# conroi/lcpc

Measured on AMD Instinct MI355X. Metric: field-elements committed/sec (whole node), Ligero 2^26 coeffs, higher is better.
Workload: dtype u32 limbs (255-bit prime field Ft255, Montgomery form)

## Files before the change

### lcpc_amd/csrc/ctx.cpp

```cpp
#include "internal.h"
#include <chrono>

using namespace lcpc;

namespace lcpc {


const uint8_t LBL_DT[7] = "$l//DT", LBL_PR[7] = "$l//PR", LBL_PE[7] = "$l//PE", LBL_CO[7] = "$l//CO";

void ctx_ref(lcpc_ctx* c) { c->refs.fetch_add(1); }

static void ctx_free(lcpc_ctx* c) {
  (void)hipSetDevice(c->prm.device);
  comm_release(c);
  for (const NttStep& s : c->ntt) dev_free(s.pack);
  dev_free(c->d_wq_w); dev_free(c->d_rootsls); dev_free(c->d_rootslcs);
  dev_free(c->d_rootsl); dev_free(c->d_rootslc); dev_free(c->d_qpl); dev_free(c->d_roots); dev_free(c->d_r2);
  dev_free(c->ws.d_tmp); dev_free(c->ws.d_t); dev_free(c->ws.d_mid); dev_free(c->d_scratch);
  c->verify_sets.clear();
  if (c->s_verify) (void)hipStreamDestroy(c->s_verify);
  for (unsigned k = 0; k < lcpc_ctx::N_STAGE; k++) {
    if (c->h_stage[k]) (void)hipHostFree(c->h_stage[k]);
    if (c->ev_stage[k]) (void)hipEventDestroy(c->ev_stage[k]);
  }
  for (auto* v : {&c->d_pre, &c->d_post})
    for (auto& d : *v) { dev_free(d.rowptr); dev_free(d.colidx); dev_free(d.vals); dev_free(d.vals29); }
  delete c;
}
void ctx_unref(lcpc_ctx* c) {
  if (c->refs.fetch_sub(1) == 1) ctx_free(c);
}

uint64_t ntt_mid_rows(const lcpc_ctx* c, uint64_t n_rows) {
  const bool ev = c->sw_ntt_mid_max_mb >= 0;
  if (c->ntt.size() != 2 || c->ntt[0].kernel != NttStep::K1S || n_rows == 0) return 0;
  if (!ev && c->log_n > 15) return 0;
  const uint64_t max_mb = ev ? (uint64_t)c->sw_ntt_mid_max_mb : 6144;
  if (max_mb == 0) return 0;
  const uint64_t per_row = c->n_cols * 36;
  uint64_t fit = (max_mb << 20) / per_row;
  if (fit == 0) return 0;
  if (fit >= n_rows) return n_rows;
  const uint64_t batches = (n_rows + fit - 1) / fit;
  return (n_rows + batches - 1) / batches;
}

static void wmul_table(const FieldDesc& f, const uint64_t* w_mont, int N, int W, uint32_t out[96]) {
  uint64_t v[MAXL];
  h_canon(f, v, w_mont);
  memset(out, 0, 96 * 4);
  for (int j = 0; j < N; j++) {
    uint64_t m[5] = {0, 0, 0, 0, 0};
    for (int i = 0; i < f.L; i++) m[i] = v[i];
    bool big = false;
    for (int i = f.L - 1; i >= 0; i--) {
      const uint64_t h = (f.p[i] >> 1) | (i + 1 < f.L ? f.p[i + 1] << 63 : 0);
      if (v[i] != h) { big = v[i] > h; break; }
    }
    if (big) {
      unsigned __int128 br = 0;
      for (int i = 0; i < 5; i++) { const unsigned __int128 d = (unsigned __int128)m[i] - (i < f.L ? f.p[i] : 0) - (uint64_t)br; m[i] = (uint64_t)d; br = (d >> 64) & 1; }
    }
    for (int k = 0; k < N; k++) {
      const int b = W * k, wd = b / 64, sh = b % 64;
      uint64_t x = m[wd] >> sh;
      if (sh && wd + 1 < 5) x |= m[wd + 1] << (64 - sh);
      out[N * k + j] = k < N - 1 ? (uint32_t)(x & (((uint64_t)1 << W) - 1)) : (uint32_t)x;
    }
    for (int s = 0; s < W; s++) h_add(f, v, v, v);
  }
}
static int build_wq_w(lcpc_ctx* c, int N, int W) {
  const FieldDesc* f = c->f;
  uint64_t i4[MAXL];
  memcpy(i4, f->rou, 8 * f->L);
  for (unsigned i = 0; i + 2 < f->S; i++) h_mul(*f, i4, i4, i4);
  uint32_t wt[96];
  wmul_table(*f, i4, N, W, wt);
  int rc = dev_alloc(&c->err, &c->d_wq_w, sizeof wt);
  if (rc) return rc;
  HIPCHK(c, hipMemcpy(c->d_wq_w, wt, sizeof wt, hipMemcpyHostToDevice));
  return 0;
}

static std::vector<uint32_t> clamp_table(const FieldDesc& f, int N, int W, int stride) {
  std::vector<uint32_t> tab((size_t)64 * stride, 0);
  for (int i = 0; i < 64; i++) {
    const int q = i - 24;
    uint64_t mag[5] = {0, 0, 0, 0, 0};
    unsigned __int128 cy = 0;
    for (int w = 0; w < 5; w++) { cy += (unsigned __int128)(w < f.L ? f.p[w] : 0) * (uint64_t)(q < 0 ? -q : q); mag[w] = (uint64_t)cy; cy >>= 64; }
    if (q < 0) {
      unsigned __int128 c2 = 1;
      for (int w = 0; w < 5; w++) { c2 += (unsigned __int128)(~mag[w]); mag[w] = (uint64_t)c2; c2 >>= 64; }
    }
    for (int l = 0; l < N; l++) {
      const int b = W * l, w = b / 64, sh = b % 64;
      uint64_t x = mag[w] >> sh;
      if (sh && w + 1 < 5) x |= mag[w + 1] << (64 - sh);
      tab[(size_t)i * stride + l] = l + 1 < N ? (uint32_t)(x & (((uint64_t)1 << W) - 1)) : (uint32_t)x;
    }
  }
  return tab;
}
static int limb_consts(lcpc_ctx* c, std::vector<uint32_t**>* made) {
  const int N = ntt_lns_limbs(c->NL), W = ntt_lns_limb_bits(c->NL);
  const std::vector<uint32_t> tab = clamp_table(*c->f, N, W, ntt_lns_stride(c->NL));
  if (made) { made->push_back(&c->d_qpl); made->push_back(&c->d_wq_w); }
  if (int rc = dev_alloc(&c->err, &c->d_qpl, tab.size() * 4)) return rc;
  HIPCHK(c, hipMemcpy(c->d_qpl, tab.data(), tab.size() * 4, hipMemcpyHostToDevice));
  return build_wq_w(c, N, W);
}

static void plan_passes(lcpc_ctx* c) {
  const unsigned k = c->log_n;
  const int NL = c->NL;
  const int lt_small = NL >= 6 ? 10 : (NL == 4 ? 11 : 12);
  const int lt_big = NL >= 6 ? 11 : 12;
  unsigned ltj_min = 0;
  while (((size_t)NL * 4 << ltj_min) < 128) ltj_min++;
  c->ntt.clear();
  auto add = [&](unsigned t0, unsigned s, unsigned log_tj, int lt) {
    NttStep p;
    p.log_tile = lt;
    p.a.roots = c->d_roots; p.a.roots29 = c->d_rootsl; p.a.qp29 = c->d_qpl; p.a.wq_w = c->d_wq_w;
    p.a.log_n = k; p.a.t0 = t0; p.a.s = s; p.a.log_tj = log_tj;
    p.roots29c = c->d_rootslc;
    p.mont_prefix = t0 + s == k ? (k == 0 ? 1u : (s % 2 == 0 ? 4u : 2u)) : 0u;
    c->ntt.push_back(p);
  };
  if ((int)k <= lt_small) {
    add(0, k, 0, lt_small);
    return;
  }
  int LT = lt_small;
  auto n_pass = [&](int lt) { unsigned per = lt - ltj_min, rest = k - lt; return 1 + (rest + per - 1) / per; };
  if (c->L == 4 && (k == 19 || k == 20) && !c->sw_ntt_general) {
    add(0, k - 10, 20 - k, 10);
    add(k - 10, 10, 0u, 10);
    return;
  }
  if (n_pass(lt_small) > 2 && n_pass(lt_big) < n_pass(lt_small)) LT = lt_big;
  const unsigned P = n_pass(LT);
  const unsigned s_final = LT;
  unsigned rem = k - s_final, t0 = 0;
  for (unsigned i = 0; i + 1 < P; i++) {
    const unsigned left = P - 1 - i;
    const unsigned s = (rem + left - 1) / left;
    add(t0, s, (uint32_t)LT - s, LT);
    t0 += s;
    rem -= s;
  }
  add(t0, s_final, 0u, LT);
}

static uint32_t ntt_tile_group_of(uint32_t log_n, int L, uint32_t log_tj) {
  const uint32_t tiles_log = log_n - 10;
  if (tiles_log < 3) return 0;
  uint32_t run_log = log_tj;
  for (uint32_t b = 8u * (uint32_t)L; b > 1; b >>= 1) run_log++;
  uint32_t lg = run_log <= 5 ? 11 - run_log : (run_log < 10 ? 10 - run_log : 0);
  return std::min(std::min(lg, 6u), tiles_log - 3);
}

static int build_limb_plan(lcpc_ctx* c, unsigned n_pass) {
  std::vector<uint32_t**> made;
  std::vector<NttStep> plan(n_pass);
  const int rc = [&]() -> int {
    const FieldDesc* f = c->f;
    ErrText* err = &c->err;
    const unsigned k = c->log_n, s0 = k - 10 * (n_pass - 1);
    const size_t stride = (size_t)ntt_lns_stride(c->NL);
    auto alloc = [&](uint32_t** p, size_t bytes) { made.push_back(p); return dev_alloc(err, p, bytes); };
    int r;
    if (c->L != 4) {
      uint64_t rp[2 * MAXL] = {1, 0, 0, 0};
      for (int i = 0; i < ntt_lns_limbs(c->NL) * ntt_lns_limb_bits(c->NL); i++) h_add(*f, rp, rp, rp);
      h_canon(*f, rp + f->L, rp);
      const size_t n_roots = (size_t)1 << (k - 1);
      uint32_t* d_rp = nullptr;
      if ((r = dev_alloc(err, &d_rp, 16 * f->L))) return r;
      if ((r = alloc(&c->d_rootsl, n_roots * stride * 4)) || (r = alloc(&c->d_rootslc, n_roots * stride * 4))) { dev_free(d_rp); return r; }
      hipError_t he = hipMemcpy(d_rp, rp, 16 * f->L, hipMemcpyHostToDevice);
      if (he == hipSuccess) he = launch_ntt_lns_roots(c->NL, c->d_roots, n_roots, d_rp, c->d_rootsl, nullptr);
      if (he == hipSuccess) he = launch_ntt_lns_roots(c->NL, c->d_roots, n_roots, d_rp + 2 * f->L, c->d_rootslc, nullptr);
      if (he == hipSuccess) he = hipDeviceSynchronize();
      dev_free(d_rp);
      if (he != hipSuccess) return fail_hip(err, he, "ntt_lns tables");
      if ((r = limb_consts(c, &made))) return r;
    }
    if (n_pass == 3) {
      const size_t n_sub = (size_t)1 << 19;
      if ((r = alloc(&c->d_rootsls, n_sub * stride * 4)) || (r = alloc(&c->d_rootslcs, n_sub * stride * 4))) return r;
      for (int i = 0; i < 2; i++) {
        const uint32_t* tab = i ? c->d_rootslc : c->d_rootsl;
        uint32_t* sub = i ? c->d_rootslcs : c->d_rootsls;
        HIPCHK(c, launch_ntt_lns_subtable(c->NL, tab, s0, n_sub, sub, nullptr));
      }
    }
    for (unsigned i = 0; i < n_pass; i++) {
      NttStep& p = plan[i];
      const bool sub = n_pass == 3 && i > 0, last = i + 1 == n_pass;
      p.kernel = c->L == 4 ? NttStep::K1S : NttStep::K1N;
      p.first = !last;
      p.a.roots = c->d_roots; p.a.roots29 = sub ? c->d_rootsls : c->d_rootsl; p.a.qp29 = c->d_qpl; p.a.wq_w = c->d_wq_w;
      p.a.log_n = sub ? 20u : k;
      p.a.t0 = last ? p.a.log_n - 10 : 0u;
      p.a.s = i == 0 ? s0 : 10u;
      p.a.log_tj = 10 - p.a.s;
      p.a.tile_group = p.first ? ntt_tile_group_of(p.a.log_n, c->L, p.a.log_tj) : 0u;
      p.a.canon_row_mask = sub ? (1u << (k - 20)) - 1 : 0u;
      p.roots29c = sub ? c->d_rootslcs : c->d_rootslc;
      p.mont_prefix = last && c->NL == 2 ? 4u : 0u;
      p.blk0_gone = last && c->NL != 2 && plan[i - 1].a.s >= 8 ? 1u : 0u;
      p.pack_info = ntt_lns_pack_info(c->NL, p.a.s, p.first);
      const uint32_t n_classes = p.first ? 1u << (p.a.log_n - 10) : 1u;
#ifdef LCPC_TEST_HOOKS
      if (n_pass == 3 && i == 0 && c->sw_test_fail_3pass) return LCPC_ERR_NOMEM;
#endif
      if ((r = alloc(&p.pack, (size_t)n_classes * p.pack_info.class_words * 4))) return r;
      NttPassArgs pa{};
      pa.roots29 = p.a.roots29; pa.roots29c = p.roots29c; pa.log_n = p.a.log_n; pa.t0 = p.a.t0; pa.s = p.a.s; pa.log_tj = p.a.log_tj;
      HIPCHK(c, launch_ntt_lns_pack(c->NL, pa, p.first, p.pack_info, n_classes, p.pack, nullptr));
    }
    HIPCHK(c, hipDeviceSynchronize());
    return 0;
  }();
  if (rc == 0) {
    c->ntt = std::move(plan);
    c->comm_canon = true;
    return 0;
  }
  for (uint32_t** p : made) { dev_free(*p); *p = nullptr; }
  if (rc != LCPC_ERR_NOMEM) return rc;
  (void)hipGetLastError();
  c->err.clear();
  return 0;
}

#define ECHK(call)                                                        \
  do {                                                                    \
    hipError_t e__ = (call);                                              \
    if (e__ != hipSuccess) return fail_hip(err, e__, #call);              \
  } while (0)

template <class Mat, class Rs> static int sdig_walk(const lcpc_ctx* c, Mat&& mat, Rs&& rs) {
  const size_t t = c->d_pre.size();
  const DevCsr& pl = c->d_pre[t - 1];
  uint64_t in_start = 0;
  for (size_t i = 0; i + 1 < t; i++) {
    if (int rc = mat(c->d_pre[i], in_start, in_start + c->d_pre[i].n_in, false)) return rc;
    in_start += c->d_pre[i].n_in;
  }
  if (int rc = mat(pl, in_start, 0, true)) return rc;
  const uint64_t in_end = in_start + pl.n_in;
  if (int rc = rs(in_end, c->d_post[t - 1].n_in)) return rc;
  in_start = in_end + pl.n_out;
  uint64_t out_start = in_end + c->d_post[t - 1].n_in;
  for (size_t ii = t; ii-- > 0;) {
    in_start -= c->d_pre[ii].n_out;
    if (int rc = mat(c->d_post[ii], in_start, out_start, false)) return rc;
    out_start += c->d_post[ii].n_out;
  }
  return 0;
}

int encode_rows_device(const lcpc_ctx* c, EncodeWs* ws, const EncodeJob& j, hipStream_t st, ErrText* err, uint32_t* launches) {
  uint32_t dummy = 0;
  uint32_t& nl = launches ? *launches : dummy;
  if (j.kept_t) *j.kept_t = false;
  const uint64_t n_rows = j.n_rows;
  if (n_rows == 0) return 0;
  if (c->prm.encoding == LCPC_ENC_LIGERO) {
    uint64_t rb = ws->mid_failed ? 0 : ntt_mid_rows(c, n_rows);
    if (rb) {
      ErrText scratch_err;
      uint64_t want = rb * c->n_cols * 36;
#ifdef LCPC_TEST_HOOKS
      if (c->sw_test_fail_mid) want = (uint64_t)1 << 62;
#endif
      if (ensure_dev(&scratch_err, &ws->d_mid, &ws->mid_cap, want)) {
        (void)hipGetLastError();
        ws->mid_failed = true; ws->mid_cap = 0; rb = 0;
      }
    }
    const uint64_t batch = rb ? rb : n_rows;
    for (uint64_t r0 = 0; r0 < n_rows; r0 += batch) {
      const uint64_t nr = std::min(batch, n_rows - r0), consumed = r0 * j.src_stride;
      for (size_t i = 0; i < c->ntt.size(); i++) {
        const NttStep& p = c->ntt[i];
        const bool first = i == 0;
        const uint64_t len = (uint64_t)1 << p.a.log_n;
        NttPassArgs a = p.a;
        if (j.canon_out) { a.roots29c = p.roots29c; a.mont_prefix = p.mont_prefix; a.blk0_gone = p.blk0_gone; }
        a.dst = j.dst + r0 * c->n_cols * c->NL;
        a.src = first ? j.src + consumed * c->NL : a.dst;
        a.src_stride = first ? j.src_stride : len;
        a.dst_stride = len;
        a.n_valid = first ? j.n_valid : len;
        a.n_src_total = !first || j.n_src_total == ~(uint64_t)0 ? ~(uint64_t)0 : (j.n_src_total > consumed ? j.n_src_total - consumed : 0);
        a.copy_dst = first && j.copy_dst ? j.copy_dst + consumed * c->NL : nullptr;
        a.n_rows = nr << (c->log_n - p.a.log_n);
        a.mid = rb ? ws->d_mid : nullptr;
        switch (p.kernel) {
          case NttStep::K1S: ECHK(launch_ntt_pass_l9s(a, p.first, p.pack, p.pack_info, st)); break;
          case NttStep::K1N: ECHK(launch_ntt_pass_lns(c->NL, a, p.first, p.pack, p.pack_info, st)); break;
          case NttStep::GENERAL: ECHK(launch_ntt_pass(c->NL, p.log_tile, a, st)); break;
        }
        nl++;
      }
    }
    return 0;
  }
  const size_t t = c->d_pre.size();
  const DevCsr& pl = c->d_pre[t - 1];
  const size_t eb = elem_bytes(c);
  if (int rc = ensure_dev(err, &ws->d_tmp, &ws->tmp_cap, n_rows * pl.n_out * eb)) return rc;
  if (n_rows >= SDIG_T_MIN_ROWS) {
    if (int rc = ensure_dev(err, &ws->d_t, &ws->t_cap, n_rows * c->n_cols * eb)) return rc;
    ECHK(launch_transpose_to_t(c->NL, j.src, j.src_stride, j.n_valid, n_rows, ws->d_t, st, j.n_src_total, j.copy_dst, j.canon_out && j.keep_t));
    nl++;
    SpmmTArgs a{};
    a.t = ws->d_t; a.n_rows = n_rows;
    auto mat = [&](const DevCsr& m, uint64_t in_off, uint64_t out_off, bool to_tmp) -> int {
      a.out_alt = to_tmp ? ws->d_tmp : nullptr; a.in_off = in_off; a.out_off = out_off;
      a.rowptr = m.rowptr; a.colidx = m.colidx; a.vals = m.vals; a.vals29 = m.vals29; a.m = m.n_out;
      ECHK(launch_spmm_t(c->NL, a, st));
      nl++;
      return 0;
    };
    auto rs = [&](uint64_t out_off, uint64_t n_out) -> int {
      ECHK(launch_sdig_rs_t(c->NL, ws->d_tmp, (uint32_t)pl.n_out, ws->d_t, out_off, (uint32_t)n_out, n_rows, c->d_r2, st));
      nl++;
      return 0;
    };
    if (int rc = sdig_walk(c, mat, rs)) return rc;
    if (j.keep_t) {
      if (j.kept_t) *j.kept_t = true;
      return 0;
    }
    ECHK(launch_transpose_from_t(c->NL, ws->d_t, c->n_cols, n_rows, j.dst, c->n_cols, st));
    nl++;
    return 0;
  }
  if (j.src != j.dst || j.src_stride != c->n_cols) {
    ECHK(launch_pad_rows(c->NL, j.src, j.src_stride, j.dst, c->n_cols, j.n_valid, n_rows, st));
    nl++;
  }
  SpmvArgs a{};
  a.mat = j.dst; a.stride = c->n_cols; a.n_rows = n_rows;
  auto mat = [&](const DevCsr& m, uint64_t in_off, uint64_t out_off, bool to_tmp) -> int {
    a.out_alt = to_tmp ? ws->d_tmp : nullptr; a.in_off = in_off; a.out_off = out_off;
    if (to_tmp) a.out_alt_stride = pl.n_out;
    a.rowptr = m.rowptr; a.colidx = m.colidx; a.vals = m.vals; a.vals29 = m.vals29; a.m = m.n_out;
    ECHK(launch_spmv(c->NL, a, st));
    nl++;
    return 0;
  };
  auto rs = [&](uint64_t out_off, uint64_t n_out) -> int {
    ECHK(launch_sdig_rs(c->NL, ws->d_tmp, pl.n_out, (uint32_t)pl.n_out, j.dst, c->n_cols, out_off, (uint32_t)n_out, n_rows, c->d_r2, st));
    nl++;
    return 0;
  };
  return sdig_walk(c, mat, rs);
}

}

extern "C" {

int lcpc_abi_version(void) { return LCPC_ABI_VERSION; }

const char* lcpc_strerror(int s) {
  switch (s) {
    case LCPC_OK: return "ok";
    case LCPC_ERR_TOO_BIG: return "n_cols is too large for this encoding";
    case LCPC_ERR_ENCODE: return "encoding error";
    case LCPC_ERR_COMMIT: return "inconsistent commitment fields";
    case LCPC_ERR_COLUMN_NUMBER: return "bad column number";
    case LCPC_ERR_OUTER_TENSOR: return "outer tensor: wrong size";
    case LCPC_ERR_DIMS: return "dimensions not valid for this encoding";
    case LCPC_ERR_ARG: return "invalid argument";
    case LCPC_ERR_STATE: return "no commitment in this object";
    case LCPC_ERR_HIP: return "HIP runtime error";
    case LCPC_ERR_NOMEM: return "out of memory";
    case LCPC_ERR_NO_DEVICE: return "no usable HIP device (this library has no CPU fallback)";
    case LCPC_ERR_XCHG: return "all-gather of the sharded commit / prove failed";
    case LCPC_ERR_NO_RCCL: return "librccl could not be loaded";
    case LCPC_VERR_NUM_COL_OPENS: return "wrong number of column openings in proof";
    case LCPC_VERR_COLUMN_PATH: return "column verification: merkle path failed";
    case LCPC_VERR_COLUMN_EVAL: return "column verification: eval dot product failed";
    case LCPC_VERR_COLUMN_DEGREE: return "column verification: degree test dot product failed";
    case LCPC_VERR_OUTER_TENSOR: return "outer tensor: wrong size";
    case LCPC_VERR_INNER_TENSOR: return "inner tensor: wrong size";
    case LCPC_VERR_ENCODING_DIMS: return "encoding dimension mismatch";
    case LCPC_VERR_ENCODE: return "encoding error";
    case LCPC_VERR_MALFORMED: return "malformed proof bytes";
  }
  return "unknown status";
}
const char* lcpc_last_error(const lcpc_ctx* c) { return c ? c->err.c_str() : ""; }

int lcpc_static_get_dims(const lcpc_params* p, uint64_t* nr, uint64_t* np, uint64_t* nc) {
  if (!p || !nr || !np || !nc) return LCPC_ERR_ARG;
  LCPC_TRY
  const FieldDesc* f = field_desc((int)p->field);
  if (!f || p->n_coeffs == 0) return LCPC_ERR_ARG;
  if (p->encoding == LCPC_ENC_LIGERO) {
    if (p->rho_num == 0 || p->rho_num >= p->rho_den) return LCPC_ERR_ARG;
    return ligero_get_dims(*f, p->n_coeffs, p->rho_num, p->rho_den, nr, np, nc) ? LCPC_ERR_TOO_BIG : 0;
  } else if (p->encoding == LCPC_ENC_SDIG) {
    SdigSpec s;
    const int code = p->sdig_code ? (int)p->sdig_code : 3;
    uint64_t npr;
    if (!sdig_spec(code, &s) || !sdig_n_per_row(*f, p->n_coeffs, code, &npr)) return LCPC_ERR_ARG;
    std::vector<LevelDims> pre, post;
    if (!sdig_level_dims(s, npr, (double)f->flog2(), pre, post)) return LCPC_ERR_DIMS;
    *nr = (p->n_coeffs + npr - 1) / npr; *np = npr; *nc = sdig_codeword_length(pre, post);
    return 0;
  }
  return LCPC_ERR_ARG;
  LCPC_CATCH((lcpc_ctx*)nullptr)
}

int lcpc_static_get_dims_ml(const lcpc_params* p, uint32_t n_vars, uint64_t* nr, uint64_t* np, uint64_t* nc) {
  if (!p || !nr || !np || !nc || n_vars >= 63) return LCPC_ERR_ARG;
  LCPC_TRY
  const FieldDesc* f = field_desc((int)p->field);
  if (!f) return LCPC_ERR_ARG;
  const uint64_t n = (uint64_t)1 << n_vars;
  if (p->encoding == LCPC_ENC_LIGERO) {
    lcpc_params q = *p;
    q.n_coeffs = n;
    int rc = lcpc_static_get_dims(&q, nr, np, nc);
    if (rc) return rc;
    if ((*nr & (*nr - 1)) || (*np & (*np - 1)) || *nr * *np != n) return LCPC_ERR_DIMS;
    return 0;
  } else if (p->encoding == LCPC_ENC_SDIG) {
    SdigSpec s;
    const int code = p->sdig_code ? (int)p->sdig_code : 3;
    uint64_t npr;
    if (!sdig_spec(code, &s) || !sdig_n_per_row(*f, n, code, &npr, true)) return LCPC_ERR_ARG;
    std::vector<LevelDims> pre, post;
    if (!sdig_level_dims(s, npr, (double)f->flog2(), pre, post)) return LCPC_ERR_DIMS;
    *nr = (n + npr - 1) / npr; *np = npr; *nc = sdig_codeword_length(pre, post);
    return 0;
  }
  return LCPC_ERR_ARG;
  LCPC_CATCH((lcpc_ctx*)nullptr)
}

static int ctx_build(lcpc_ctx* c, const lcpc_params* p) {
  const FieldDesc* f = c->f;
  ErrText* err = &c->err;
  int rc = 0;
  if (p->encoding == LCPC_ENC_LIGERO) {
    if (p->rho_num == 0 || p->rho_num >= p->rho_den) return LCPC_ERR_ARG;
    uint64_t nr, np_, nc;
    if (p->n_per_row && p->n_cols) { np_ = p->n_per_row; nc = p->n_cols; }
    else if ((rc = lcpc_static_get_dims(p, &nr, &np_, &nc))) return rc;
    if (!(np_ < nc) || (nc & (nc - 1)) || log2_ceil(nc) > f->S) return LCPC_ERR_DIMS;
    if (log2_ceil(nc) > 30) return LCPC_ERR_TOO_BIG;
    c->n_per_row = np_; c->n_cols = nc; c->log_n = (unsigned)log2_ceil(nc);
    {
      const unsigned log_half = c->log_n ? c->log_n - 1 : 0;
      const size_t n_roots = (size_t)1 << log_half;
      std::vector<uint64_t> pw((size_t)(log_half + 1) * f->L);
      uint64_t w[MAXL];
      memcpy(w, f->rou, 8 * f->L);
      for (unsigned i = 0; i < f->S - c->log_n; i++) h_mul(*f, w, w, w);
      for (unsigned j = 0; j <= log_half; j++) { memcpy(&pw[(size_t)j * f->L], w, 8 * f->L); h_mul(*f, w, w, w); }
      uint32_t *d_pw = nullptr, *d_one = nullptr;
      if ((rc = dev_alloc(err, &d_pw, pw.size() * 8)) || (rc = dev_alloc(err, &d_one, 8 * f->L)) ||
          (rc = dev_alloc(err, &c->d_roots, n_roots * 8 * f->L)) ||
          (f->L == 4 && (rc = dev_alloc(err, &c->d_rootsl, n_roots * 48))) ||
          (f->L == 4 && (rc = dev_alloc(err, &c->d_rootslc, n_roots * 48)))) {
        dev_free(d_pw); dev_free(d_one);
        return rc;
      }
      hipError_t he = hipMemcpy(d_pw, pw.data(), pw.size() * 8, hipMemcpyHostToDevice);
      if (he == hipSuccess) he = hipMemcpy(d_one, f->r, 8 * f->L, hipMemcpyHostToDevice);
      if (he == hipSuccess) he = launch_roots(c->NL, d_pw, log_half, d_one, c->d_roots, c->d_rootsl, c->d_rootslc, nullptr);
      if (he == hipSuccess) he = hipDeviceSynchronize();
      dev_free(d_pw); dev_free(d_one);
      if (he != hipSuccess) return fail_hip(err, he, "precomp_fft");
    }
    if (f->L == 4) {
      if ((rc = limb_consts(c, nullptr))) return rc;
      c->comm_canon = true;
    }
    if ((rc = dev_alloc(err, &c->d_r2, 8 * f->L))) return rc;
    HIPCHK(c, hipMemcpy(c->d_r2, f->r2, 8 * f->L, hipMemcpyHostToDevice));
    plan_passes(c);
    if (c->sw_ntt_general) return 0;
    const uint32_t np = (uint32_t)c->ntt.size();
    if (c->L == 4 ? ntt_l9s_supported(c->log_n, np, c->ntt[0].log_tile) : np >= 2 && ntt_lns_supported(c->NL, c->log_n)) return build_limb_plan(c, 2);
    if (c->L == 4 ? ntt_l9s3_supported(c->log_n) : np >= 2 && ntt_lns3_supported(c->NL, c->log_n)) return build_limb_plan(c, 3);
    return 0;
  }
  if (p->encoding != LCPC_ENC_SDIG) return LCPC_ERR_ARG;
  if (!sdig_spec((int)c->prm.sdig_code, &c->spec)) return LCPC_ERR_ARG;
  uint64_t npr = p->n_per_row;
  if (!(p->n_per_row && p->n_cols)) {
    if (!sdig_n_per_row(*f, p->n_coeffs, (int)c->prm.sdig_code, &npr)) return LCPC_ERR_ARG;
  }
  std::vector<CsrMatrix> pre, post;
  const bool dbg = c->sw_debug_timing;
  auto now = [] { return std::chrono::duration<double, std::milli>(std::chrono::steady_clock::now().time_since_epoch()).count(); };
  const double t_gen0 = now();
  if (!sdig_generate(*f, c->spec, npr, p->seed, pre, post, c->pre_dims, c->post_dims)) return LCPC_ERR_DIMS;
  const double t_gen1 = now();
  c->n_per_row = npr;
  c->n_cols = sdig_codeword_length(c->pre_dims, c->post_dims);
  if (p->n_per_row && p->n_cols && p->n_cols != c->n_cols) return LCPC_ERR_DIMS;
  uint32_t* d_rprime = nullptr;
  if (f->L == 2 || f->L == 3) {
    uint64_t rp[MAXL] = {1, 0, 0, 0};
    for (int i = 0; i < ntt_lns_limbs(c->NL) * ntt_lns_limb_bits(c->NL); i++) h_add(*f, rp, rp, rp);
    if ((rc = dev_alloc(err, &d_rprime, 8 * f->L))) return rc;
    HIPCHK(c, hipMemcpy(d_rprime, rp, 8 * f->L, hipMemcpyHostToDevice));
  }
  struct FreeRp { uint32_t*& p; ~FreeRp() { if (p) { (void)hipDeviceSynchronize(); dev_free(p); p = nullptr; } } } free_rp{d_rprime};
  auto upload = [&](const CsrMatrix& m, DevCsr& d) -> int {
    d.n_in = m.n_in; d.n_out = m.n_out;
    int r;
    if ((r = dev_alloc(err, &d.rowptr, m.rowptr.size() * 4))) return r;
    if ((r = dev_alloc(err, &d.colidx, m.colidx.size() * 4))) return r;
    if ((r = dev_alloc(err, &d.vals, m.vals.size() * 8))) return r;
    HIPCHK(c, hipMemcpy(d.rowptr, m.rowptr.data(), m.rowptr.size() * 4, hipMemcpyHostToDevice));
    HIPCHK(c, hipMemcpy(d.colidx, m.colidx.data(), m.colidx.size() * 4, hipMemcpyHostToDevice));
    HIPCHK(c, hipMemcpy(d.vals, m.vals.data(), m.vals.size() * 8, hipMemcpyHostToDevice));
    if (f->L == 4) {
      const size_t nnz = m.colidx.size();
      if ((r = dev_alloc(err, &d.vals29, (nnz + 1) * 48))) return r;
      HIPCHK(c, launch_to_r29(d.vals, nnz, d.vals29, nullptr));
      HIPCHK(c, hipMemsetAsync(d.vals29 + nnz * 12, 0, 48, nullptr));
    } else if ((f->L == 2 || f->L == 3) && d_rprime) {
      const size_t nnz = m.colidx.size();
      const size_t stride = (size_t)ntt_lns_stride(c->NL);
      if ((r = dev_alloc(err, &d.vals29, (nnz + 1) * stride * 4))) return r;
      HIPCHK(c, launch_ntt_lns_roots(c->NL, d.vals, nnz, d_rprime, d.vals29, nullptr));
      HIPCHK(c, hipMemsetAsync(d.vals29 + nnz * stride, 0, stride * 4, nullptr));
    }
    return 0;
  };
  c->d_pre.resize(pre.size());
  c->d_post.resize(post.size());
  for (size_t i = 0; i < pre.size() && !rc; i++) { rc = upload(pre[i], c->d_pre[i]); if (!rc) rc = upload(post[i], c->d_post[i]); }
  if (!rc) rc = dev_alloc(err, &c->d_r2, 8 * f->L);
  if (rc) return rc;
  HIPCHK(c, hipMemcpy(c->d_r2, f->r2, 8 * f->L, hipMemcpyHostToDevice));
  if (dbg) fprintf(stderr, "[SdigEncoding::new] matgen %.1f ms, convert + upload %.1f ms\n", t_gen1 - t_gen0, now() - t_gen1);
  return 0;
}

int lcpc_ctx_create(const lcpc_params* p, lcpc_ctx** out) {
  if (!p || !out) return LCPC_ERR_ARG;
  *out = nullptr;
  lcpc_ctx* c = nullptr;
  LCPC_TRY
  const FieldDesc* f = field_desc((int)p->field);
  if (!f || p->hash > LCPC_HASH_SHA256) return LCPC_ERR_ARG;
  if (p->hash != LCPC_HASH_BLAKE3 && p->shard_count > 1) return LCPC_ERR_ARG;
  int ndev = 0;
  if (hipGetDeviceCount(&ndev) != hipSuccess || ndev <= 0 || p->device < 0 || p->device >= ndev) return LCPC_ERR_NO_DEVICE;
  if (hipSetDevice(p->device) != hipSuccess) return LCPC_ERR_NO_DEVICE;
  c = new lcpc_ctx();
  c->prm = *p;
  c->f = f; c->L = f->L; c->NL = 2 * f->L;
  if (c->prm.sdig_code == 0) c->prm.sdig_code = 3;
  c->sw_ntt_general = getenv("LCPC_NTT_GENERAL") != nullptr;
  if (const char* ev = getenv("LCPC_NTT_MID_MAX_MB")) c->sw_ntt_mid_max_mb = (int64_t)strtoull(ev, nullptr, 10);
  if (const char* ev = getenv("LCPC_HOST_STAGE")) c->sw_host_stage = (int32_t)strtol(ev, nullptr, 10);
  c->sw_debug_timing = getenv("LCPC_DEBUG_TIMING") != nullptr;
#ifdef LCPC_TEST_HOOKS
  if (const char* ev = getenv("LCPC_TEST_FAIL")) {
    c->sw_test_fail_3pass = strstr(ev, "3pass") != nullptr;
    c->sw_test_fail_mid = strstr(ev, "mid") != nullptr;
  }
#endif
  int rc = 0;
  if (c->prm.shard_count > 1 && c->prm.shard_rank >= c->prm.shard_count) rc = LCPC_ERR_ARG;
  if (!rc) rc = ctx_build(c, p);
  if (rc) { ctx_unref(c); return rc; }
  c->np2 = next_pow2(c->n_cols);
  c->path_len = (uint32_t)log2_ceil(c->n_cols);
  if (c->sw_host_stage > 0) {
    c->stage_cap = (size_t)64 << 20;
    for (unsigned k = 0; k < 2; k++) {
      if (hipHostMalloc(reinterpret_cast<void**>(&c->h_stage[k]), c->stage_cap, hipHostMallocDefault) != hipSuccess) { (void)hipGetLastError(); c->h_stage[k] = nullptr; break; }
      if (hipEventCreateWithFlags(&c->ev_stage[k], hipEventDisableTiming) != hipSuccess) { (void)hipGetLastError(); (void)hipHostFree(c->h_stage[k]); c->h_stage[k] = nullptr; c->ev_stage[k] = nullptr; break; }
    }
  }
  *out = c;
  return 0;
  } catch (...) {
    if (c) ctx_unref(c);
    return LCPC_ERR_NOMEM;
  }
}

void lcpc_ctx_destroy(lcpc_ctx* c) {
  if (c) ctx_unref(c);
}

int lcpc_get_dims(const lcpc_ctx* c, uint64_t len, uint64_t* nr, uint64_t* np, uint64_t* nc) {
  if (!c || len == 0) return LCPC_ERR_ARG;
  if (nr) *nr = (len + c->n_per_row - 1) / c->n_per_row;
  if (np) *np = c->n_per_row;
  if (nc) *nc = c->n_cols;
  return 0;
}
int lcpc_dims_ok(const lcpc_ctx* c, uint64_t n_per_row, uint64_t n_cols) {
  if (!c) return 0;
  bool ok = n_per_row < n_cols && n_per_row == c->n_per_row && n_cols == c->n_cols;
  if (c->prm.encoding == LCPC_ENC_LIGERO) ok = ok && (n_cols & (n_cols - 1)) == 0;
  return ok ? 1 : 0;
}
uint64_t lcpc_get_n_col_opens(const lcpc_ctx* c) {
  if (!c) return 0;
  return c->prm.encoding == LCPC_ENC_LIGERO ? ligero_n_col_opens(c->prm.rho_num, c->prm.rho_den) : sdig_n_col_opens((int)c->prm.sdig_code);
}
uint64_t lcpc_get_n_degree_tests(const lcpc_ctx* c) { return c ? n_degree_tests(128, c->n_cols, c->f->flog2()) : 0; }
uint32_t lcpc_field_limbs(const lcpc_ctx* c) { return c ? (uint32_t)c->L : 0; }

int lcpc_encode_rows(lcpc_ctx* c, uint64_t* rows, uint64_t n_rows) {
  if (!c || !rows) return LCPC_ERR_ARG;
  if (n_rows == 0) return 0;
  LCPC_TRY
  std::lock_guard<std::mutex> g(c->mu);
  HIPCHK(c, hipSetDevice(c->prm.device));
  const size_t bytes = (size_t)n_rows * c->n_cols * elem_bytes(c);
  int rc = ensure_dev(&c->err, &c->d_scratch, &c->scratch_cap, bytes);
  if (rc) return rc;
  HIPCHK(c, hipMemcpy(c->d_scratch, rows, bytes, hipMemcpyHostToDevice));
  EncodeJob j;
  j.src = c->d_scratch; j.src_stride = c->n_cols; j.n_valid = c->n_cols; j.dst = c->d_scratch; j.n_rows = n_rows;
  if ((rc = encode_rows_device(c, &c->ws, j, nullptr, &c->err, nullptr))) return rc;
  HIPCHK(c, hipMemcpy(rows, c->d_scratch, bytes, hipMemcpyDeviceToHost));
  return 0;
  LCPC_CATCH(c)
}

}

namespace lcpc {
int encode_msgs_host(lcpc_ctx* c, const uint64_t* const* msgs, uint64_t n_rows, uint64_t* out) {
  if (n_rows == 0) return 0;
  std::lock_guard<std::mutex> g(c->mu);
  HIPCHK(c, hipSetDevice(c->prm.device));
  if (!c->s_verify) HIPCHK(c, hipStreamCreateWithFlags(&c->s_verify, hipStreamNonBlocking));
  hipStream_t st = c->s_verify;
  struct Drain { hipStream_t st; ~Drain() { (void)hipStreamSynchronize(st); } } drain{st};
  const size_t eb = elem_bytes(c);
  const size_t in_b = ((size_t)n_rows * c->n_per_row * eb + 255) & ~(size_t)255, out_b = (size_t)n_rows * c->n_cols * eb;
  int rc = ensure_dev(&c->err, &c->d_scratch, &c->scratch_cap, in_b + out_b);
  if (rc) return rc;
  uint8_t* base = reinterpret_cast<uint8_t*>(c->d_scratch);
  for (uint64_t i = 0; i < n_rows; i++)
    HIPCHK(c, hipMemcpyAsync(base + i * c->n_per_row * eb, msgs[i], c->n_per_row * eb, hipMemcpyHostToDevice, st));
  EncodeJob j;
  j.src = reinterpret_cast<uint32_t*>(base); j.src_stride = c->n_per_row; j.n_valid = c->n_per_row;
  j.dst = reinterpret_cast<uint32_t*>(base + in_b); j.n_rows = n_rows;
  if ((rc = encode_rows_device(c, &c->ws, j, st, &c->err, nullptr))) return rc;
  HIPCHK(c, hipMemcpyAsync(out, base + in_b, out_b, hipMemcpyDeviceToHost, st));
  HIPCHK(c, hipStreamSynchronize(st));
  return 0;
}
}

extern "C" {

int lcpc_field_sum_device(lcpc_ctx* c, const uint64_t* parts, uint32_t n_parts, uint64_t n_elems, void* stream, uint64_t* out) {
  if (!c || !parts || !out || n_parts == 0) return LCPC_ERR_ARG;
  hipError_t he = hipSetDevice(c->prm.device);
  if (he == hipSuccess)
    he = launch_field_sum(c->NL, reinterpret_cast<const uint32_t*>(parts), n_parts, n_elems, reinterpret_cast<uint32_t*>(out), (hipStream_t)stream);
  if (he != hipSuccess) {
    std::lock_guard<std::mutex> g(c->mu);
    return fail_hip(&c->err, he, "lcpc_field_sum_device");
  }
  return 0;
}

void lcpc_root_bincode(const uint8_t root[32], uint8_t out[40]) {
  const uint64_t l = 32;
  memcpy(out, &l, 8);
  memcpy(out + 8, root, 32);
}
void lcpc_free(void* p) { lcpc::proof_buf_free(p); }

}
```

### lcpc_amd/csrc/internal.h

```cpp
#pragma once
#include "../../include/lcpc_hip.h"
#include <hip/hip_runtime.h>
#include <stdio.h>
#include <stdlib.h>
#include <string.h>
#include <algorithm>
#include <atomic>
#include <condition_variable>
#include <memory>
#include <mutex>
#include <new>
#include <shared_mutex>
#include <string>
#include <thread>
#include <vector>
#include "encoding.h"
#include "host_crypto.h"
#include "host_field.h"
#include "host_par.h"
#include "kernels.h"

namespace lcpc {

struct DevCsr {
  uint64_t n_in = 0, n_out = 0;
  uint32_t *rowptr = nullptr, *colidx = nullptr, *vals = nullptr;
  uint32_t* vals29 = nullptr;
};
struct NttStep {
  enum Kernel { GENERAL, K1S, K1N } kernel = GENERAL;
  bool first = false;
  int log_tile = 0;
  NttPassArgs a{};
  const uint32_t* roots29c = nullptr;
  uint32_t mont_prefix = 0, blk0_gone = 0;
  uint32_t* pack = nullptr;
  NttPackInfo pack_info{};
};

struct EncodeWs {
  uint32_t* d_tmp = nullptr;
  uint64_t tmp_cap = 0;
  uint32_t* d_t = nullptr;
  uint64_t t_cap = 0;
  uint32_t* d_mid = nullptr;
  uint64_t mid_cap = 0;
  bool mid_failed = false;
};
uint64_t ntt_mid_rows(const lcpc_ctx* c, uint64_t n_rows);

constexpr uint64_t SDIG_T_MIN_ROWS = 24;

void* proof_buf_alloc(size_t n);
void proof_buf_free(void* p);

class ErrText {
 public:
  ErrText& operator=(const std::string& s) { set(s.c_str()); return *this; }
  ErrText& operator=(const char* s) { set(s); return *this; }
  void clear() { set(""); }
  const char* c_str() const { return buf_[cur_.load(std::memory_order_acquire)]; }
 private:
  void set(const char* s) {
    std::lock_guard<std::mutex> g(mu_);
    const unsigned k = (cur_.load(std::memory_order_relaxed) + 1) % 4;
    snprintf(buf_[k], sizeof buf_[k], "%s", s ? s : "");
    cur_.store(k, std::memory_order_release);
  }
  std::mutex mu_;
  std::atomic<unsigned> cur_{0};
  char buf_[4][512] = {};
};

class FillLock {
 public:
  void lock() {
    std::unique_lock<std::mutex> g(mu_);
    ++fills_waiting_;
    cv_.wait(g, [&] { return !filling_ && readers_ == 0; });
    --fills_waiting_;
    filling_ = true;
  }
  void unlock() {
    { std::lock_guard<std::mutex> g(mu_); filling_ = false; }
    cv_.notify_all();
  }
  void lock_shared() {
    std::unique_lock<std::mutex> g(mu_);
    cv_.wait(g, [&] { return !filling_ && fills_waiting_ == 0; });
    ++readers_;
  }
  void unlock_shared() {
    bool last;
    { std::lock_guard<std::mutex> g(mu_); last = --readers_ == 0; }
    if (last) cv_.notify_all();
  }
 private:
  std::mutex mu_;
  std::condition_variable cv_;
  unsigned readers_ = 0, fills_waiting_ = 0;
  bool filling_ = false;
};

struct DevScratch {
  uint32_t* d = nullptr;
  uint64_t cap = 0;
  uint32_t* t29 = nullptr;
  uint64_t t29_cap = 0;
  void release() { if (d) (void)hipFree(d); if (t29) (void)hipFree(t29); d = t29 = nullptr; cap = t29_cap = 0; }
};

struct CallSet {
  bool busy = false;
  uint8_t* h_pin = nullptr;
  uint64_t h_pin_cap = 0;
  hipStream_t st = nullptr;
  hipEvent_t ev_slice[2] = {nullptr, nullptr};
  DevScratch sc;
  int make();
  void quiesce() { (void)hipStreamSynchronize(st); }
  ~CallSet();
};
struct VerifySet {
  bool busy = false;
  uint8_t* h_pin = nullptr;
  uint64_t h_pin_cap = 0;
  int make() { return 0; }
  void quiesce() {}
  ~VerifySet() { if (h_pin) (void)hipHostFree(h_pin); }
};

template <typename S> class SetPool {
 public:
  static constexpr size_t MAX_SETS = 8;
  int take(uint64_t pin_bytes, S** out) {
    *out = nullptr;
    std::unique_lock<std::mutex> lk(mu_);
    bool reuse_only = false;
    for (;;) {
      S* pick = nullptr;
      for (auto& s : sets_) if (!s->busy && s->h_pin_cap >= pin_bytes) { pick = s.get(); break; }
      if (!pick && !reuse_only) {
        for (auto& s : sets_) if (!s->busy) { pick = s.get(); break; }
        if (!pick && sets_.size() < MAX_SETS) {
          std::unique_ptr<S> s(new S());
          if (int rc = s->make()) return rc;
          sets_.push_back(std::move(s));
          pick = sets_.back().get();
        }
      }
      if (!pick) {
        if (reuse_only && !any_holds(pin_bytes)) return LCPC_ERR_NOMEM;
        cv_.wait(lk);
        continue;
      }
      pick->busy = true;
      if (pick->h_pin_cap >= pin_bytes) { *out = pick; return 0; }
      lk.unlock();
      if (pick->h_pin) (void)hipHostFree(pick->h_pin);
      pick->h_pin = nullptr; pick->h_pin_cap = 0;
      void* hp = nullptr;
      const bool ok = hipHostMalloc(&hp, (size_t)pin_bytes, hipHostMallocDefault) == hipSuccess;
      if (!ok) (void)hipGetLastError();
      lk.lock();
      if (ok) { pick->h_pin = static_cast<uint8_t*>(hp); pick->h_pin_cap = pin_bytes; *out = pick; return 0; }
      pick->busy = false;
      if (!any_holds(pin_bytes)) return LCPC_ERR_NOMEM;
      reuse_only = true;
    }
  }
  void give(S* s) {
    { std::lock_guard<std::mutex> g(mu_); s->busy = false; }
    cv_.notify_all();
  }
  void clear() { sets_.clear(); }
 private:
  bool any_holds(uint64_t pin_bytes) const {
    for (auto& s : sets_) if (s->h_pin_cap >= pin_bytes) return true;
    return false;
  }
  std::mutex mu_;
  std::condition_variable cv_;
  std::vector<std::unique_ptr<S>> sets_;
};
template <typename S> struct SetLease {
  SetPool<S>& pool;
  S* s = nullptr;
  ~SetLease() { if (s) { s->quiesce(); pool.give(s); } }
};

struct BatchSlab {
  uint8_t* d = nullptr;
  uint64_t off_comm = 0, off_coeffs = 0, off_hashes = 0, off_cvs = 0;
  uint64_t comm_stride = 0, coeffs_stride = 0, hashes_stride = 0, cvs_stride = 0;
  uint32_t n_batch = 0;
  uint64_t n_rows = 0;
  uint32_t* h_roots = nullptr;
  uint32_t* d_roots_alias = nullptr;
  EncodeWs ws;
  uint32_t* seg(uint64_t off, uint64_t stride, uint32_t i) const { return reinterpret_cast<uint32_t*>(d + off) + (size_t)i * stride; }
  ~BatchSlab() {
    if (d) (void)hipFree(d);
    if (ws.d_mid) (void)hipFree(ws.d_mid);
    if (h_roots) (void)hipHostFree(h_roots);
  }
};

}

struct lcpc_transcript {
  lcpc::Transcript t;
  lcpc_transcript(const uint8_t* l, size_t n) : t(l, n) {}
};

struct lcpc_ctx {
  lcpc_params prm{};
  bool sw_ntt_general = false;
  int64_t sw_ntt_mid_max_mb = -1;
  bool sw_debug_timing = false;
  bool sw_test_fail_3pass = false;
  bool sw_test_fail_mid = false;
  const lcpc::FieldDesc* f = nullptr;
  int L = 0, NL = 0;
  uint64_t n_per_row = 0, n_cols = 0, np2 = 0;
  uint32_t path_len = 0;
  unsigned log_n = 0;
  uint32_t* d_roots = nullptr;
  uint32_t* d_rootsl = nullptr;
  uint32_t* d_rootslc = nullptr;
  uint32_t* d_qpl = nullptr;
  uint32_t* d_rootsls = nullptr;
  uint32_t* d_rootslcs = nullptr;
  uint32_t* d_wq_w = nullptr;
  std::vector<lcpc::NttStep> ntt;
  bool comm_canon = false;
  lcpc::SdigSpec spec{};
  std::vector<lcpc::LevelDims> pre_dims, post_dims;
  std::vector<lcpc::DevCsr> d_pre, d_post;
  uint32_t* d_r2 = nullptr;
  lcpc::EncodeWs ws;
  uint32_t* d_scratch = nullptr;
  uint64_t scratch_cap = 0;
  void* comm = nullptr;
  std::mutex xchg_mu;
  hipEvent_t ev_xchg = nullptr;
  std::atomic<int> refs{1};
  lcpc::ErrText err;
  std::mutex mu;
  lcpc::SetPool<lcpc::VerifySet> verify_sets;
  hipStream_t s_verify = nullptr;
  std::mutex stage_mu;
  static constexpr unsigned N_STAGE = 4;
  uint8_t* h_stage[N_STAGE] = {nullptr, nullptr, nullptr, nullptr};
  hipEvent_t ev_stage[N_STAGE] = {nullptr, nullptr, nullptr, nullptr};
  size_t stage_cap = 0;
  unsigned stage_next = 0;
  int32_t sw_host_stage = -1;
};

struct lcpc_commit_s {
  lcpc_ctx* enc = nullptr;
  bool committed = false;
  uint64_t n_rows = 0;
  uint64_t row_begin = 0, n_rows_local = 0;
  uint64_t chunk_begin = 0, chunk_end = 0, n_chunks = 0;
  uint32_t *d_coeffs = nullptr, *d_comm = nullptr, *d_hashes = nullptr, *d_cvs = nullptr;
  const uint32_t* coeffs_view = nullptr;
  uint64_t cap_coeff_rows = 0, cap_comm_rows = 0, cap_cvs = 0;
  std::shared_ptr<lcpc::BatchSlab> slab;
  uint32_t slab_index = 0;
  uint32_t* d_chain = nullptr;
  uint64_t cap_chain = 0;
  lcpc::EncodeWs ws;
  bool comm_t = false;
  bool comm_rows_valid = false;
  uint32_t* d_node_tab = nullptr;
  uint64_t node_tab_key = 0;
  std::vector<uint32_t> node_slot_h, node_log_h;
  struct NodeTab { uint64_t key; uint32_t* d; std::vector<uint32_t> slot, lg; };
  std::vector<NodeTab> node_tabs;
  uint8_t* d_gather = nullptr;
  uint64_t gather_cap = 0;
  uint8_t *d_xsend = nullptr, *d_xrecv = nullptr;
  uint64_t xchg_cap = 0;
  lcpc::DevScratch sc;
  uint32_t* h_root = nullptr;
  uint32_t* d_root_alias = nullptr;
  bool timing = false;
  hipEvent_t ev[6] = {nullptr, nullptr, nullptr, nullptr, nullptr, nullptr};
  hipStream_t s_prove = nullptr;
  hipEvent_t ev_done = nullptr;
  hipStream_t s_xchg = nullptr;
  hipEvent_t ev_hashed = nullptr;
  bool shard_encoded = false;
  hipStream_t s_copy = nullptr, s_comp = nullptr;
  hipEvent_t ev_batch[16] = {nullptr};
  mutable lcpc::FillLock fill_mu;
  lcpc::SetPool<lcpc::CallSet> sets;
  std::mutex shard_prove_mu;
  lcpc_timings last{};
  uint32_t launches[3] = {0, 0, 0};
  lcpc::ErrText err;
  std::mutex mu;
};

namespace lcpc {

inline int fail_hip(ErrText* err, hipError_t e, const char* what) {
  if (err) *err = std::string(what) + ": " + hipGetErrorString(e);
  return e == hipErrorOutOfMemory ? LCPC_ERR_NOMEM : LCPC_ERR_HIP;
}
#define HIPCHK(c, call)                                                   \
  do {                                                                    \
    hipError_t e__ = (call);                                              \
    if (e__ != hipSuccess) return lcpc::fail_hip((c) ? &(c)->err : nullptr, e__, #call); \
  } while (0)

#define LCPC_TRY try {
#define LCPC_CATCH(c)                                                     \
  } catch (const std::bad_alloc&) {                                       \
    if (c) (c)->err = "host allocation failed";                          \
    return LCPC_ERR_NOMEM;                                                \
  } catch (const std::exception& ex__) {                                  \
    if (c) (c)->err = ex__.what();                                       \
    return LCPC_ERR_STATE;                                                \
  } catch (...) {                                                         \
    return LCPC_ERR_STATE;                                                \
  }

template <typename T> int dev_alloc(ErrText* err, T** p, size_t bytes) {
  *p = nullptr;
  if (bytes == 0) bytes = 16;
  hipError_t e = hipMalloc(reinterpret_cast<void**>(p), bytes);
  if (e != hipSuccess) return fail_hip(err, e, "hipMalloc");
  return 0;
}
inline void dev_free(void* p) { if (p) (void)hipFree(p); }
template <typename T> int ensure_dev(ErrText* err, T** p, uint64_t* cap, uint64_t bytes) {
  bytes = (bytes + 255) & ~(uint64_t)255;
  if (bytes > *cap || !*p) {
    dev_free(*p);
    *p = nullptr; *cap = 0;
    int rc = dev_alloc(err, p, (size_t)bytes);
    if (rc) return rc;
    *cap = bytes;
  }
  return 0;
}

inline size_t elem_bytes(const lcpc_ctx* c) { return (size_t)8 * c->L; }
inline bool is_sha3(const lcpc_ctx* c) { return c->prm.hash == LCPC_HASH_SHA3_256; }
inline bool is_blake2b(const lcpc_ctx* c) { return c->prm.hash == LCPC_HASH_BLAKE2B; }
inline bool is_keccak256(const lcpc_ctx* c) { return c->prm.hash == LCPC_HASH_KECCAK256; }
inline bool is_sha256(const lcpc_ctx* c) { return c->prm.hash == LCPC_HASH_SHA256; }
inline bool is_blake3(const lcpc_ctx* c) { return c->prm.hash == LCPC_HASH_BLAKE3; }
inline uint32_t digest_len(const lcpc_ctx* c) { return is_blake2b(c) ? 64u : 32u; }
inline uint32_t digest_words(const lcpc_ctx* c) { return digest_len(c) / 4; }
inline uint64_t leaf_chunks(const lcpc_ctx* c, uint64_t n_rows) { return (32 + elem_bytes(c) * n_rows + 1023) / 1024; }

extern const uint8_t LBL_DT[7], LBL_PR[7], LBL_PE[7], LBL_CO[7];


void ctx_ref(lcpc_ctx* c);
void ctx_unref(lcpc_ctx* c);
struct EncodeJob {
  const uint32_t* src = nullptr;
  uint64_t src_stride = 0, n_valid = 0;
  uint32_t* dst = nullptr;
  uint64_t n_rows = 0;
  uint64_t n_src_total = ~(uint64_t)0;
  uint32_t* copy_dst = nullptr;
  bool canon_out = false;
  bool keep_t = false;
  bool* kept_t = nullptr;
};
int encode_rows_device(const lcpc_ctx* c, EncodeWs* ws, const EncodeJob& j, hipStream_t st, ErrText* err, uint32_t* launches);

int encode_msgs_host(lcpc_ctx* c, const uint64_t* const* msgs, uint64_t n_rows, uint64_t* out);

int ensure_scratch(lcpc_commit_t* m, DevScratch* sc, uint64_t bytes);
int ensure_cvs(lcpc_commit_t* m, uint64_t n_chunks);
int begin_commit(lcpc_commit_t* m, hipStream_t st, uint64_t n_rows_total, uint64_t row_begin, uint64_t row_end, uint64_t chunk_begin,
                 uint64_t chunk_end);
int ensure_commit_buffers(lcpc_commit_t* m, uint64_t n_rows_local, bool own_coeffs, bool comm_rows);
void leave_slab(lcpc_commit_t* m);
int commit_device_locked(lcpc_commit_t* m, const uint64_t* coeffs_dev, uint64_t n_coeffs, hipStream_t st, uint32_t flags, uint8_t* root);
int encode_coeffs(lcpc_commit_t* m, const uint32_t* src, uint64_t n_src, bool borrow, hipStream_t st);
int hash_chunks(lcpc_commit_t* m, uint64_t a, uint64_t b, uint32_t* out, hipStream_t st);
int merkle_top(lcpc_commit_t* m, hipStream_t st, uint32_t levels_done = 0);
int seal_commit(lcpc_commit_t* m, hipStream_t st, uint8_t* root);
int order_after_commit(lcpc_commit_t* m, hipStream_t st);
int collapse_run(lcpc_commit_t* m, DevScratch* sc, const uint32_t* d_tensors, uint32_t n_tensors, hipStream_t st, uint32_t* d_polys);
size_t collapse_scratch_bytes(const lcpc_commit_t* m, uint32_t n_tensors);
int take_call_set(lcpc_commit_t* m, uint64_t pin_bytes, CallSet** ws);
int collapse_host(lcpc_commit_t* m, CallSet* ws, const uint64_t* tensors, uint32_t n_tensors, uint64_t* polys, uint64_t* polys_canon);
int collapse_host_sliced(lcpc_commit_t* m, CallSet* ws, const uint64_t* tensor, uint64_t* polys, uint64_t* polys_canon, uint64_t* cut_out);
int collapse_wait_slice(lcpc_commit_t* m, CallSet* ws, int s);
int open_columns_host(lcpc_commit_t* m, CallSet* ws, const uint64_t* cols, uint32_t n, uint64_t* col_vals, size_t vals_pitch, uint8_t* paths);
int open_columns_device(lcpc_commit_t* m, const uint64_t* d_cols, uint32_t n, uint32_t* d_vals, uint32_t* d_paths, hipStream_t st);

void shard_layout_of(const lcpc_ctx* c, uint64_t g, uint64_t n_rows, uint64_t* rb, uint64_t* re, uint64_t* cb, uint64_t* ce, uint64_t* nch);
int shard_nodes(uint64_t c0, uint64_t c1, uint64_t* first, uint32_t* lg);
void shard_chunk_range(uint64_t F, uint64_t n_chunks, uint64_t G, uint64_t g, uint64_t* c0, uint64_t* c1);
void comm_release(lcpc_ctx* c);
struct ShardXchg {
  uint8_t *send_dev, *recv_dev;
  uint64_t max_bytes;
  lcpc_allgather_fn fn;
  void* user;
  bool stream_ordered = false;
};
int prove_stream(lcpc_commit_t* m, hipStream_t* st);
int collapse_sharded(lcpc_commit_t* m, const ShardXchg& x, const uint64_t* tensors_full, uint32_t nt, uint64_t* polys, uint64_t* polys_canon);
int open_sharded(lcpc_commit_t* m, const ShardXchg& x, const uint64_t* cols, uint32_t n, uint64_t* vals, size_t vals_pitch, uint8_t* paths);

int prove_impl(lcpc_commit_t* m, const uint64_t* outer, uint64_t n_outer, lcpc_transcript* trw, uint8_t** proof, uint64_t* proof_len,
               uint64_t* cols_opened, const ShardXchg* xchg);

}
```

### lcpc_amd/csrc/kernels.h

```cpp
#pragma once
#include <hip/hip_runtime.h>
#include <stdint.h>

namespace lcpc {

struct NttPassArgs {
  const uint32_t* src;
  uint32_t* dst;
  const uint32_t* roots;
  const uint32_t* roots29;
  const uint32_t* qp29;
  const uint32_t* roots29c;
  uint32_t mont_prefix;
  uint64_t src_stride, dst_stride;
  uint64_t n_valid;
  uint64_t n_src_total;
  uint32_t* copy_dst;
  uint64_t n_rows;
  uint32_t log_n, t0, s, log_tj;
  uint32_t* mid = nullptr;
  uint32_t canon_row_mask = 0;
  uint32_t blk0_gone = 0;
  const uint32_t* wq_w = nullptr;
  uint32_t tile_group = 0;
};
hipError_t launch_ntt_pass(int nl, int log_tile, const NttPassArgs& a, hipStream_t st);

struct NttPackInfo {
  uint32_t round_off[8];
  uint32_t class_words;
  uint32_t u_off;
};
bool ntt_l9s_supported(uint32_t log_n, uint32_t n_passes, int log_tile);
bool ntt_l9s3_supported(uint32_t log_n);
hipError_t launch_ntt_pass_l9s(const NttPassArgs& a, bool first, const uint32_t* pack, const NttPackInfo& pi, hipStream_t st);

bool ntt_lns_supported(int nl, uint32_t log_n);
bool ntt_lns3_supported(int nl, uint32_t log_n);
hipError_t launch_ntt_pass_lns(int nl, const NttPassArgs& a, bool first, const uint32_t* pack, const NttPackInfo& pi, hipStream_t st);
int ntt_lns_limbs(int nl);
int ntt_lns_limb_bits(int nl);
int ntt_lns_stride(int nl);
hipError_t launch_ntt_lns_subtable(int nl, const uint32_t* tab, uint32_t shift, uint64_t n, uint32_t* sub, hipStream_t st);
NttPackInfo ntt_lns_pack_info(int nl, uint32_t s, bool first);
hipError_t launch_ntt_lns_roots(int nl, const uint32_t* roots, uint64_t n, const uint32_t* rprime, uint32_t* out, hipStream_t st);
hipError_t launch_ntt_lns_pack(int nl, const NttPassArgs& a, bool first, const NttPackInfo& pi, uint32_t n_classes, uint32_t* pack, hipStream_t st);

hipError_t launch_roots(int nl, const uint32_t* pw, uint32_t log_half, const uint32_t* one, uint32_t* roots, uint32_t* roots29,
                        uint32_t* roots29c, hipStream_t st);

struct LeafArgs {
  const uint32_t* comm;
  uint64_t row_stride;
  uint64_t col_stride;
  uint64_t n_cols;
  int64_t  row_base;
  uint64_t n_rows_total;
  uint32_t chunk_begin, n_chunks_local, n_chunks_total;
  uint32_t* out;
  uint32_t canon_in;
};
hipError_t launch_leaf_chunks(int nl, const LeafArgs& a, hipStream_t st);
hipError_t launch_leaf_finish(uint32_t* cvs, uint32_t n_chunks, uint64_t n_cols, uint32_t* digests, hipStream_t st);
hipError_t launch_leaf_finish_nodes(uint32_t* cvs, const uint32_t* node_slot, const uint32_t* node_log, uint32_t n_nodes,
                                    uint64_t n_cols, uint32_t* out, bool root, hipStream_t st);
hipError_t launch_merkle_tree(uint32_t* hashes, uint64_t np2, hipStream_t st, uint32_t* root_out);
hipError_t launch_merkle_tree_from(uint32_t* hashes, uint64_t np2, uint32_t levels_done, hipStream_t st, uint32_t* root_out);
bool leaf_tree_supported(const LeafArgs& a, uint64_t np2);
hipError_t launch_leaf_tree(int nl, const LeafArgs& a, uint32_t* hashes, uint64_t np2, hipStream_t st);

hipError_t launch_leaf_chunks_batch(int nl, const LeafArgs& a, uint32_t n_batch, uint64_t comm_stride, uint64_t out_stride, hipStream_t st);
hipError_t launch_leaf_finish_batch(uint32_t* cvs, uint32_t n_chunks, uint64_t n_cols, uint32_t* digests, uint32_t n_batch, uint64_t cvs_stride,
                                    uint64_t digests_stride, hipStream_t st);
hipError_t launch_leaf_tree_batch(int nl, const LeafArgs& a, uint32_t* hashes, uint64_t np2, uint32_t n_batch, uint64_t comm_stride,
                                  uint64_t hashes_stride, hipStream_t st);
hipError_t launch_merkle_tree_from_batch(uint32_t* hashes, uint64_t np2, uint32_t levels_done, uint32_t n_batch, uint64_t hashes_stride,
                                         hipStream_t st, uint32_t* root_out);
hipError_t launch_batch_place(const uint64_t* src, uint64_t src_stride, uint64_t n_valid, uint64_t* dst, uint64_t dst_stride, uint32_t n_batch,
                              hipStream_t st);

hipError_t launch_sha3_leaves(int nl, const LeafArgs& a, hipStream_t st);
hipError_t launch_sha3_merkle_tree(uint32_t* hashes, uint64_t np2, hipStream_t st, uint32_t* root_out);
hipError_t launch_keccak256_leaves(int nl, const LeafArgs& a, hipStream_t st);
hipError_t launch_keccak256_merkle_tree(uint32_t* hashes, uint64_t np2, hipStream_t st, uint32_t* root_out);

hipError_t launch_sha256_leaves(int nl, const LeafArgs& a, hipStream_t st);
hipError_t launch_sha256_merkle_tree(uint32_t* hashes, uint64_t np2, hipStream_t st, uint32_t* root_out);

hipError_t launch_blake2b_leaves(int nl, const LeafArgs& a, hipStream_t st);
hipError_t launch_blake2b_merkle_tree(uint32_t* hashes, uint64_t np2, hipStream_t st, uint32_t* root_out);
hipError_t launch_blake2b_gather_paths(const uint32_t* hashes, uint64_t np2, uint32_t path_len, const uint64_t* cols, uint32_t n,
                                       uint32_t* paths, hipStream_t st);

inline uint64_t sha3_leaf_blocks(int nl, uint64_t n_rows_total) { return (4 + (uint64_t)(nl / 2) * n_rows_total) / 17 + 1; }
inline uint64_t sha256_leaf_blocks(int nl, uint64_t n_rows_total) {
  const uint64_t w = 4 + (uint64_t)(nl / 2) * n_rows_total;
  return w / 8 + 1 + ((w & 7) == 7 ? 1 : 0);
}
inline uint64_t blake2b_leaf_blocks(int nl, uint64_t n_rows_total) { return (8 + (uint64_t)(nl / 2) * n_rows_total + 15) / 16; }
constexpr uint32_t SHA3_STATE_WORDS = 50, SHA256_STATE_WORDS = 8, BLAKE2B_STATE_WORDS = 16;
hipError_t launch_sha3_leaves_range(int nl, const LeafArgs& a, uint64_t blk_begin, uint64_t blk_end, uint64_t* state, hipStream_t st);
hipError_t launch_keccak256_leaves_range(int nl, const LeafArgs& a, uint64_t blk_begin, uint64_t blk_end, uint64_t* state, hipStream_t st);
hipError_t launch_sha256_leaves_range(int nl, const LeafArgs& a, uint64_t blk_begin, uint64_t blk_end, uint32_t* state, hipStream_t st);
hipError_t launch_blake2b_leaves_range(int nl, const LeafArgs& a, uint64_t blk_begin, uint64_t blk_end, uint64_t* state, hipStream_t st);

struct CollapseArgs {
  const uint32_t* coeffs;
  const uint32_t* tensors;
  const uint32_t* tensors29;
  uint32_t* out;
  uint64_t n_rows, n_per_row;
  uint32_t n_tensors, n_splits;
  uint64_t j0 = 0, j1 = 0, out_stride = 0;
};
hipError_t launch_collapse(int nl, const CollapseArgs& a, hipStream_t st);
hipError_t launch_to_r29(const uint32_t* in, uint64_t n, uint32_t* out, hipStream_t st);
hipError_t launch_field_sum(int nl, const uint32_t* parts, uint32_t n_parts, uint64_t n_elems, uint32_t* out, hipStream_t st);

hipError_t launch_gather_columns(int nl, const uint32_t* comm, uint64_t n_rows, uint64_t row_stride, uint64_t col_stride,
                                 const uint64_t* cols, uint32_t n, uint32_t* vals, const uint32_t* r2, hipStream_t st);
hipError_t launch_to_mont(int nl, const uint32_t* in, uint64_t n, const uint32_t* r2, uint32_t* out, hipStream_t st);
hipError_t launch_to_canon(int nl, const uint32_t* in, uint64_t n, uint32_t* out, hipStream_t st);
hipError_t launch_assemble_columns(int nl, const uint32_t* recv, uint64_t block_words, const uint64_t* rb, uint32_t G, uint32_t n,
                                   uint64_t n_rows, uint32_t* out, hipStream_t st);
hipError_t launch_gather_paths(const uint32_t* hashes, uint64_t np2, uint32_t path_len, const uint64_t* cols, uint32_t n,
                               uint32_t* paths, hipStream_t st);

struct SpmvArgs {
  uint32_t* mat;
  uint32_t* out_alt;
  uint64_t stride, out_alt_stride;
  uint64_t in_off, out_off;
  const uint32_t* rowptr;
  const uint32_t* colidx;
  const uint32_t* vals;
  const uint32_t* vals29;
  uint64_t m, n_rows;
};
hipError_t launch_spmv(int nl, const SpmvArgs& a, hipStream_t st);
hipError_t launch_transpose_to_t(int nl, const uint32_t* src, uint64_t src_stride, uint64_t n_valid, uint64_t n_rows,
                                 uint32_t* t, hipStream_t st, uint64_t n_src_total = ~(uint64_t)0, uint32_t* copy_dst = nullptr,
                                 bool canon = false);
hipError_t launch_transpose_from_t(int nl, const uint32_t* t, uint64_t n_pos, uint64_t n_rows, uint32_t* dst,
                                   uint64_t dst_stride, hipStream_t st);
struct SpmmTArgs {
  uint32_t* t;
  uint32_t* out_alt;
  uint64_t n_rows;
  uint64_t in_off, out_off;
  const uint32_t* rowptr;
  const uint32_t* colidx;
  const uint32_t* vals;
  const uint32_t* vals29;
  uint64_t m;
};
hipError_t launch_spmm_t(int nl, const SpmmTArgs& a, hipStream_t st);
hipError_t launch_sdig_rs_t(int nl, const uint32_t* in_t, uint32_t n_in, uint32_t* t, uint64_t out_off, uint32_t n_out,
                            uint64_t n_rows, const uint32_t* r2, hipStream_t st);

hipError_t launch_sdig_rs(int nl, const uint32_t* in, uint64_t in_stride, uint32_t n_in, uint32_t* mat, uint64_t stride,
                          uint64_t out_off, uint32_t n_out, uint64_t n_rows, const uint32_t* r2, hipStream_t st);
hipError_t launch_pad_rows(int nl, const uint32_t* src, uint64_t src_stride, uint32_t* dst, uint64_t dst_stride,
                           uint64_t n_valid, uint64_t n_rows, hipStream_t st);

}
```

### lcpc_amd/csrc/ntt_l9s.hip

```cpp
#include "kernels.h"
#include "ntt_ln_dev.h"

namespace lcpc {

namespace {

template <int S, int LTJ, bool FIRST, bool MID>
__global__ void __launch_bounds__(256, 4) ntt_pass_l9s_kernel(NttPassArgs a, const u32* __restrict__ pack, NttPackInfo pi) {
  using FT = LnField<FT255>;
  constexpr int NL = 8, LT = S + LTJ, LBT = LTJ;
  constexpr bool LAST = !FIRST;
  static_assert(LT == 10, "1024-element tiles: one radix-4 quad (two radix-2 pairs) per thread and round");
  static_assert(FIRST || (LTJ == 0 && S % 2 == 0), "the last pass works on contiguous tiles and ends with the trivial stages k-2, k-1");
  using SH = Shape<S, LBT>;
  constexpr int RU = SH::RU;
  auto SWZ = [](u32 e) -> u32 { if constexpr (RU >= 0) return e ^ ((e >> 4) & 15u); else return e; };
  extern __shared__ __attribute__((aligned(16))) u32 lds[];
  constexpr u32 T = 1u << LT;
  u32* nqp = lds + (size_t)T * 9;
  const u32 k = a.log_n;
  const u32 tiles_per_row = 1u << (k - LT);
  u64 row;
  u32 tile;
  if (FIRST && a.tile_group) {
    const u32 lg = a.tile_group;
    const u32 xcd = blockIdx.x & 7u;
    const u64 qq = blockIdx.x >> 3;
    const u32 sub = (u32)qq & ((1u << lg) - 1);
    const u64 q2 = qq >> lg;
    tile = (((u32)(q2 / a.n_rows) * 8u + xcd) << lg) | sub;
    row = q2 % a.n_rows;
  } else if (tiles_per_row >= 8) {
    const u32 xcd = blockIdx.x & 7u;
    const u64 qq = blockIdx.x >> 3;
    tile = (u32)(qq / a.n_rows) * 8u + xcd;
    row = qq % a.n_rows;
  } else {
    row = blockIdx.x / tiles_per_row;
    tile = blockIdx.x % tiles_per_row;
  }
  const u32 tid = threadIdx.x;
  mem_phase(true);
  const u32 lb = FIRST ? k - S : 0u;
  auto gindex = [&](u32 e) -> u32 {
    if constexpr (FIRST) return ((e >> LBT) << lb) | (tile << LTJ) | (e & ((1u << LBT) - 1));
    else return (tile << S) | e;
  };
  const bool canon = a.roots29c != nullptr && ((u32)row & a.canon_row_mask) == 0;
  for (u32 i = tid; i < 64 * 12; i += 256) nqp[i] = 0u - a.qp29[i];
  const u32* src = a.src + row * a.src_stride * NL;
  constexpr bool DIRECT = !(LAST && MID);
  LN<9> xin[4];
  if constexpr (LAST && MID) {
    const uint4* t4 = reinterpret_cast<const uint4*>(a.mid + (row << k) * 9 + (size_t)tile * (9 * T));
    uint4* l4 = reinterpret_cast<uint4*>(lds);
    if constexpr (RU >= 0) {
#pragma unroll
      for (u32 i = tid; i < 2 * T; i += 256) l4[(i & ~(T - 1)) | SWZ(i & (T - 1))] = t4[i];
#pragma unroll
      for (u32 i = tid; i < T / 4; i += 256) {
        const uint4 v = t4[2 * T + i];
        const u32 b = 8 * T + SWZ(4 * i);
        lds[b] = v.x; lds[b ^ 1u] = v.y; lds[b ^ 2u] = v.z; lds[b ^ 3u] = v.w;
      }
    } else {
#pragma unroll
    for (u32 i = tid; i < 9 * T / 4; i += 256) l4[i] = t4[i];
    }
  } else {
#pragma unroll
  for (u32 it = 0; it < 4; it++) {
    const u32 e = tid + 256u * it;
    const u32 g = gindex(e);
    Fe<NL> v;
    if constexpr (FIRST) {
      v = (g < a.n_valid && row * a.src_stride + g < a.n_src_total) ? fe_load<NL>(src + (size_t)g * NL) : fe_zero<NL>();
      if (a.copy_dst != nullptr && g < a.n_valid) fe_store<NL>(a.copy_dst + (row * a.src_stride + g) * NL, v);
    } else {
      v = fe_load<NL>(src + (size_t)g * NL);
    }
    xin[it] = ln::from_packed<FT>(v);
  }
  __builtin_amdgcn_sched_barrier(0);
  }
  const u32* cls_pack = pack + (size_t)(FIRST ? tile : 0u) * pi.class_words;
  const bool blk0_tile = (FIRST || tile == 0) && a.blk0_gone == 0;
  const bool zero_hi = FIRST && a.n_valid <= (1ull << (k - 1));
  if constexpr (!DIRECT) __syncthreads();

  if constexpr (SH::U0 == 1) {
    constexpr u32 half = 1u << (S - 1 + LBT);
    const u32* blk = cls_pack + pi.round_off[0];
#pragma unroll
    for (u32 pp = 0; pp < 2; pp++) {
      const u32 e1 = tid + 256u * pp;
      const LN<9> w = pack_get<FT, 2>(blk, SH::period2, canon ? 1u : 0u, e1);
      const LN<9> x = DIRECT ? xin[pp] : planes_get<FT>(lds, T, SWZ(e1));
      if (pp == 0) mem_phase(false);
      if (zero_hi) {
        if constexpr (DIRECT) planes_put<FT>(lds, T, SWZ(e1), x);
        planes_put<FT>(lds, T, SWZ(e1 + half), ln::mul<FT>(x, w));
      } else {
        const LN<9> y = DIRECT ? xin[pp + 2] : planes_get<FT>(lds, T, SWZ(e1 + half));
        LN<9> sum = ln::add(x, y);
        ln::normalize<FT>(sum);
        planes_put<FT>(lds, T, SWZ(e1), sum);
        planes_put<FT>(lds, T, SWZ(e1 + half), ln::mul<FT>(ln::sub(x, y), w));
      }
    }
    mem_phase(true);
    __syncthreads();
  }

  const u32 q = tid;
#pragma unroll
  for (int r = 0; r < SH::NR4; r++) {
    const int u = SH::U0 + 2 * r, hb = S - u - 1;
    const bool last_two = LAST && (r == SH::NR4 - 1);
    const u32 lp = q & ((1u << LBT) - 1), j = q >> LBT;
    const u32 i0 = ((j >> (hb - 1)) << (hb + 1)) | (j & ((1u << (hb - 1)) - 1));
    const u32 e0 = (i0 << LBT) | lp;
    constexpr u32 one = 1u;
    const u32 dq = one << (hb - 1 + LBT);
    const u32 period = one << (hb - 1 + LBT);
    const u32 jl = q & (period - 1);
    const u32* blk = cls_pack + pi.round_off[SH::U0 + r];
    if constexpr (RU >= 0) {
      if (r >= RU && !last_two) {
        const u32 wv = __builtin_amdgcn_readfirstlane(tid >> 6);
        const u32 qu = ((tid & 63u) << 2) | wv;
        const u32 lpu = qu & ((1u << LBT) - 1), ju = qu >> LBT;
        const u32 iu = ((ju >> (hb - 1)) << (hb + 1)) | (ju & ((1u << (hb - 1)) - 1));
        const u32 eu = (iu << LBT) | lpu;
        const u32* wu = cls_pack + pi.u_off + ((r - RU) * 4 + wv) * (3 * U_SLOT<FT>);
        const LN<9> x0 = planes_get<FT>(lds, T, SWZ(eu)), x1 = planes_get<FT>(lds, T, SWZ(eu + dq));
        const LN<9> x2 = planes_get<FT>(lds, T, SWZ(eu + 2 * dq)), x3 = planes_get<FT>(lds, T, SWZ(eu + 3 * dq));
        mem_phase(false);
        const LN<9> b0 = ln::add(x0, x2), b1 = ln::add(x1, x3);
        LN<9> c0 = ln::add(b0, b1);
        ln::clamp_apply<FT>(c0, ln::clamp_row<FT>(nqp, ln::clamp_q<FT>(c0.v[8])));
        planes_put<FT>(lds, T, SWZ(eu), c0);
        LN<9> d1 = ln::sub(b0, b1);
        ln::normalize<FT>(d1);
        planes_put<FT>(lds, T, SWZ(eu + dq), ln::mul_u<FT>(d1, wu + 2 * U_SLOT<FT>));
        const LN<9> b2 = ln::mul_u<FT>(ln::sub(x0, x2), wu);
        const LN<9> b3 = ln::mul_u<FT>(ln::sub(x1, x3), wu + U_SLOT<FT>);
        LN<9> c2 = ln::add(b2, b3);
        ln::normalize<FT>(c2);
        planes_put<FT>(lds, T, SWZ(eu + 2 * dq), c2);
        planes_put<FT>(lds, T, SWZ(eu + 3 * dq), ln::mul_u<FT>(ln::sub(b2, b3), wu + 2 * U_SLOT<FT>));
        mem_phase(true);
        __syncthreads();
        continue;
      }
    }
    if (u == 0 && zero_hi) {
      const u32 vb = canon ? 3u : 0u;
      const LN<9> w0 = pack_get<FT, 6>(blk, period, vb + 0, jl), w3 = pack_get<FT, 6>(blk, period, vb + 1, jl), w2 = pack_get<FT, 6>(blk, period, vb + 2, jl);
      mem_phase(false);
      if (a.n_valid <= (1ull << (k - 2))) {
        const LN<9> x0 = DIRECT ? xin[0] : planes_get<FT>(lds, T, SWZ(e0));
        if constexpr (DIRECT) planes_put<FT>(lds, T, SWZ(e0), x0);
        planes_put<FT>(lds, T, SWZ(e0 + dq), ln::mul<FT>(x0, w2));
        planes_put<FT>(lds, T, SWZ(e0 + 2 * dq), ln::mul<FT>(x0, w0));
        planes_put<FT>(lds, T, SWZ(e0 + 3 * dq), ln::mul<FT>(x0, w3));
      } else {
        const LN<9> x0 = DIRECT ? xin[0] : planes_get<FT>(lds, T, SWZ(e0)), x1 = DIRECT ? xin[1] : planes_get<FT>(lds, T, SWZ(e0 + dq));
        LN<9> c0 = ln::add(x0, x1);
        ln::normalize<FT>(c0);
        planes_put<FT>(lds, T, SWZ(e0), c0);
        planes_put<FT>(lds, T, SWZ(e0 + dq), ln::mul<FT>(ln::sub(x0, x1), w2));
        const LN<9> t = ln::mul_u<FT>(x1, a.wq_w);
        planes_put<FT>(lds, T, SWZ(e0 + 2 * dq), ln::mul<FT>(ln::add(x0, t), w0));
        planes_put<FT>(lds, T, SWZ(e0 + 3 * dq), ln::mul<FT>(ln::sub(x0, t), w3));
      }
      mem_phase(true);
      __syncthreads();
      continue;
    }
    const bool from_regs = DIRECT && SH::U0 == 0 && r == 0;
    const LN<9> x0 = from_regs ? xin[0] : planes_get<FT>(lds, T, SWZ(e0)), x1 = from_regs ? xin[1] : planes_get<FT>(lds, T, SWZ(e0 + dq));
    const LN<9> x2 = from_regs ? xin[2] : planes_get<FT>(lds, T, SWZ(e0 + 2 * dq)), x3 = from_regs ? xin[3] : planes_get<FT>(lds, T, SWZ(e0 + 3 * dq));
    mem_phase(false);
    const LN<9> b0 = ln::add(x0, x2), b1 = ln::add(x1, x3);
    LN<9> c0 = ln::add(b0, b1);
    if (last_two) {
      ln::normalize<FT>(c0);
      LN<9> c1 = ln::sub(b0, b1);
      const LN<9> b2 = ln::sub(x0, x2);
      const LN<9> b3 = ln::mul_u<FT>(ln::sub(x1, x3), a.wq_w);
      LN<9> c2 = ln::add(b2, b3);
      LN<9> c3 = ln::sub(b2, b3);
      ln::normalize<FT>(c1); ln::normalize<FT>(c2); ln::normalize<FT>(c3);
      mem_phase(true);
      u32* dstq = a.dst + row * a.dst_stride * NL + (size_t)((tile << S) | e0) * NL;
      LN<9> cc[4] = {c0, c1, c2, c3};
#pragma unroll
      for (int c = 0; c < 4; c++) {
        LN<9> x = cc[c];
        ln::clamp_apply<FT>(x, ln::clamp_row<FT>(nqp, ln::clamp_q<FT>(x.v[8])));
        u32 w[8];
        ln::to_packed<FT>(w, x.v);
        Fe<NL> v;
#pragma unroll
        for (int i = 0; i < 8; i++) v.v[i] = w[i];
        if (__any((int)(x.v[8] >= FT::limb(8)))) v = fe_reduce_once<8>(w);
        fe_store<NL>(dstq + (size_t)c * NL, v);
      }
      return;
    } else {
      if (from_regs) ln::normalize<FT>(c0);
      else ln::clamp_apply<FT>(c0, ln::clamp_row<FT>(nqp, ln::clamp_q<FT>(c0.v[8])));
      planes_put<FT>(lds, T, SWZ(e0), c0);
      const bool blk0c = canon && blk0_tile && q < period && (RU < 0 || r < RU);
      if constexpr (RU >= 1) {
        if (r == RU - 1 && blk0c) {
          LN<9> k32;
#pragma unroll
          for (int i = 0; i < 9; i++) k32.v[i] = i == 0 ? 32u : 0u;
          planes_put<FT>(lds, T, SWZ(e0), ln::mul<FT>(c0, k32));
        }
      }
      const u32 vb = blk0c ? 3u : 0u;
      const LN<9> w0 = pack_get<FT, 6>(blk, period, vb + 0, jl), w3 = pack_get<FT, 6>(blk, period, vb + 1, jl);
      const LN<9> w2 = pack_get<FT, 6>(blk, period, vb + 2, jl);
      const LN<9> d1 = ln::sub(b0, b1);
      planes_put<FT>(lds, T, SWZ(e0 + dq), ln::mul<FT>(d1, w2));
      const LN<9> t = ln::mul_u<FT>(ln::sub(x1, x3), a.wq_w);
      const LN<9> e2 = ln::sub(x0, x2);
      planes_put<FT>(lds, T, SWZ(e0 + 2 * dq), ln::mul<FT>(ln::add(e2, t), w0));
      planes_put<FT>(lds, T, SWZ(e0 + 3 * dq), ln::mul<FT>(ln::sub(e2, t), w3));
    }
    mem_phase(true);
    __syncthreads();
  }

  if constexpr (FIRST && MID) {
    u32* mrow = a.mid + (row << k) * 9;
#pragma unroll
    for (u32 e = tid; e < T; e += 256) {
      const u32 e2 = (tile << LTJ) | (e & ((1u << LBT) - 1));
      u32* t = mrow + (size_t)(e >> LBT) * (9 * T);
      const LN<9> x = planes_get<FT>(lds, T, SWZ(e));
      *reinterpret_cast<uint4*>(t + (size_t)e2 * 4) = make_uint4(x.v[0], x.v[1], x.v[2], x.v[3]);
      *reinterpret_cast<uint4*>(t + (size_t)(T + e2) * 4) = make_uint4(x.v[4], x.v[5], x.v[6], x.v[7]);
      t[(size_t)8 * T + e2] = x.v[8];
    }
    return;
  }
  if constexpr (FIRST) {
  u32* dst = a.dst + row * a.dst_stride * NL;
#pragma unroll
  for (u32 e = tid; e < T; e += 256) {
    const u32 g = gindex(e);
    LN<9> x = planes_get<FT>(lds, T, SWZ(e));
    ln::clamp_apply<FT>(x, ln::clamp_row<FT>(nqp, ln::clamp_q<FT>(x.v[8])));
    u32 w[8];
    ln::to_packed<FT>(w, x.v);
    Fe<NL> v;
#pragma unroll
    for (int i = 0; i < 8; i++) v.v[i] = w[i];
    fe_store<NL>(dst + (size_t)g * NL, v);
  }
  }
}

template <int S, int LTJ, bool FIRST, bool MID>
hipError_t launch_tm(const NttPassArgs& a, const u32* pack, const NttPackInfo& pi, hipStream_t st) {
  constexpr int LT = S + LTJ;
  const u64 tiles = ((u64)1 << (a.log_n - LT)) * a.n_rows;
  const size_t lds_bytes = (((size_t)1 << LT) * 9 + 64 * LnField<FT255>::STRIDE) * 4;
  hipError_t e = hipFuncSetAttribute(reinterpret_cast<const void*>(&ntt_pass_l9s_kernel<S, LTJ, FIRST, MID>),
                                     hipFuncAttributeMaxDynamicSharedMemorySize, (int)lds_bytes);
  if (e != hipSuccess) return e;
  hipLaunchKernelGGL((ntt_pass_l9s_kernel<S, LTJ, FIRST, MID>), dim3((unsigned)tiles), dim3(256), lds_bytes, st, a, pack, pi);
  return hipGetLastError();
}
template <int S, int LTJ, bool FIRST>
hipError_t launch_t(const NttPassArgs& a, const u32* pack, const NttPackInfo& pi, hipStream_t st) {
  return a.mid ? launch_tm<S, LTJ, FIRST, true>(a, pack, pi, st) : launch_tm<S, LTJ, FIRST, false>(a, pack, pi, st);
}

}

bool ntt_l9s3_supported(uint32_t log_n) { return log_n >= 21 && log_n <= 26; }

bool ntt_l9s_supported(uint32_t log_n, uint32_t n_passes, int log_tile) { return n_passes == 2 && log_tile == 10 && log_n >= 11 && log_n <= 20; }

#define L9S_FIRST_CASES(X) X(1) X(2) X(3) X(4) X(5) X(6) X(7) X(8) X(9) X(10)

hipError_t launch_ntt_pass_l9s(const NttPassArgs& a, bool first, const uint32_t* pack, const NttPackInfo& pi, hipStream_t st) {
  if (!first) {
    if (a.s != 10 || a.log_tj != 0 || a.t0 + a.s != a.log_n) return hipErrorInvalidValue;
    if (a.mont_prefix) return hipErrorInvalidValue;
    return launch_t<10, 0, false>(a, pack, pi, st);
  }
  if (a.t0 != 0 || a.s + a.log_tj != 10 || (a.s + 10 != a.log_n && a.s + 20 != a.log_n)) return hipErrorInvalidValue;
  if (a.tile_group && ((1u << (a.log_n - 10)) >> a.tile_group) < 8) return hipErrorInvalidValue;
  switch (a.s) {
#define X(SV) case SV: return launch_t<SV, 10 - SV, true>(a, pack, pi, st);
    L9S_FIRST_CASES(X)
#undef X
  }
  return hipErrorInvalidValue;
}

}
```

### lcpc_amd/csrc/ntt_ln_dev.h

```cpp
#pragma once
#include "field_ln.h"

namespace lcpc {

template <int S, int LBT> struct Shape {
  static constexpr int U0 = S & 1;
  static constexpr int NR4 = S / 2;
  static constexpr u32 period2 = 1u << (S - 1 + LBT);
  static constexpr u32 period4(int r) { return 1u << (S - U0 - 2 * r - 2 + LBT); }
  static constexpr int RU = NR4 >= 4 ? 3 : -1;
  static constexpr int NRU = RU < 0 ? 0 : NR4 - RU;
};
template <class FT> constexpr u32 U_SLOT = (FT::N * FT::N + 31) & ~31u;
template <class FT> constexpr u32 U_ALIGN = FT::N == 9 ? 4u : 16u;

template <class FT, class C = u32> LCPC_DEV LN<FT::N> planes_get(const u32* base, C cnt, u32 e) {
  constexpr int N = FT::N;
  LN<N> r;
  if constexpr (N == 3) {
    const uint2 a = *reinterpret_cast<const uint2*>(base + (size_t)e * 2);
    r.v[0] = a.x; r.v[1] = a.y; r.v[2] = base[(size_t)cnt * 2 + e];
  } else {
    const uint4 a = *reinterpret_cast<const uint4*>(base + (size_t)e * 4);
    r.v[0] = a.x; r.v[1] = a.y; r.v[2] = a.z; r.v[3] = a.w;
    if constexpr (N == 5) {
      r.v[4] = base[(size_t)cnt * 4 + e];
    } else if constexpr (N == 7) {
      const uint2 b = *reinterpret_cast<const uint2*>(base + (size_t)cnt * 4 + (size_t)e * 2);
      r.v[4] = b.x; r.v[5] = b.y; r.v[6] = base[(size_t)cnt * 6 + e];
    } else {
      const uint4 b = *reinterpret_cast<const uint4*>(base + ((size_t)cnt + e) * 4);
      r.v[4] = b.x; r.v[5] = b.y; r.v[6] = b.z; r.v[7] = b.w; r.v[8] = base[(size_t)cnt * 8 + e];
    }
  }
  return r;
}
template <class FT, class C = u32> LCPC_DEV void planes_put(u32* base, C cnt, u32 e, const LN<FT::N>& x) {
  constexpr int N = FT::N;
  if constexpr (N == 3) {
    *reinterpret_cast<uint2*>(base + (size_t)e * 2) = make_uint2(x.v[0], x.v[1]);
    base[(size_t)cnt * 2 + e] = x.v[2];
  } else {
    *reinterpret_cast<uint4*>(base + (size_t)e * 4) = make_uint4(x.v[0], x.v[1], x.v[2], x.v[3]);
    if constexpr (N == 5) {
      base[(size_t)cnt * 4 + e] = x.v[4];
    } else if constexpr (N == 7) {
      *reinterpret_cast<uint2*>(base + (size_t)cnt * 4 + (size_t)e * 2) = make_uint2(x.v[4], x.v[5]);
      base[(size_t)cnt * 6 + e] = x.v[6];
    } else {
      *reinterpret_cast<uint4*>(base + ((size_t)cnt + e) * 4) = make_uint4(x.v[4], x.v[5], x.v[6], x.v[7]);
      base[(size_t)cnt * 8 + e] = x.v[8];
    }
  }
}

template <class FT> LCPC_DEV LN<FT::N> tab_entry(const u32* tab, u32 idx) {
  if constexpr (FT::STRIDE == 12) {
    return ln::load_limbs<FT::N>(tab + (size_t)idx * 12);
  } else {
    LN<FT::N> t;
#pragma unroll
    for (int k = 0; k < FT::N; k++) t.v[k] = tab[(size_t)idx * FT::STRIDE + k];
    return t;
  }
}

template <class FT, u32 NV> LCPC_DEV LN<FT::N> pack_get(const u32* blk, u32 period, u32 variant, u32 jl) {
  if constexpr (FT::N == 9) {
    const char* base = reinterpret_cast<const char*>(blk);
    const uint4 a = *reinterpret_cast<const uint4*>(base + (((variant * 2 + 0) * period + jl) << 4));
    const uint4 b = *reinterpret_cast<const uint4*>(base + (((variant * 2 + 1) * period + jl) << 4));
    const u32 c = *reinterpret_cast<const u32*>(base + ((NV * 2 * period * 4 + variant * period + jl) << 2));
    LN<9> t;
    t.v[0] = a.x; t.v[1] = a.y; t.v[2] = a.z; t.v[3] = a.w; t.v[4] = b.x; t.v[5] = b.y; t.v[6] = b.z; t.v[7] = b.w; t.v[8] = c;
    return t;
  } else {
    return planes_get<FT>(blk, NV * period, variant * period + jl);
  }
}
template <class FT, u32 NV> LCPC_DEV void pack_put(u32* blk, u32 period, u32 variant, u32 jl, const LN<FT::N>& x) {
  if constexpr (FT::N == 9) {
    *reinterpret_cast<uint4*>(blk + ((size_t)(variant * 2 + 0) * period + jl) * 4) = make_uint4(x.v[0], x.v[1], x.v[2], x.v[3]);
    *reinterpret_cast<uint4*>(blk + ((size_t)(variant * 2 + 1) * period + jl) * 4) = make_uint4(x.v[4], x.v[5], x.v[6], x.v[7]);
    blk[(size_t)NV * 2 * period * 4 + (size_t)variant * period + jl] = x.v[8];
  } else {
    planes_put<FT>(blk, NV * period, variant * period + jl, x);
  }
}

}
```

### lcpc_amd/csrc/ntt_lns.hip

```cpp
#include "kernels.h"
#include "ntt_ln_dev.h"

namespace lcpc {

namespace {

template <class FT> LCPC_DEV LN<FT::N> mul_i(const LN<FT::N>& x, const NttPassArgs& a) {
  if constexpr (ln::has_mul_u<FT>) return ln::mul_u<FT>(x, a.wq_w);
  else return ln::mul<FT>(x, tab_entry<FT>(a.roots29, 1u << (a.log_n - 2)));
}

constexpr u32 TILE = 1024;

template <class FT, int S, int LTJ, bool FIRST>
__global__ void __launch_bounds__(256, FT::WAVES) ntt_pass_lns_kernel(NttPassArgs a, const u32* __restrict__ pack, NttPackInfo pi) {
  constexpr int N = FT::N, NL = FT::NL, LBT = LTJ;
  constexpr bool LAST = !FIRST;
  static_assert(S + LTJ == 10, "1024-element tiles: one radix-4 quad (two radix-2 pairs) per thread and round");
  static_assert(FIRST || (LTJ == 0 && S % 2 == 0), "the last pass works on contiguous tiles and ends with the trivial stages k-2, k-1");
  using SH = Shape<S, LBT>;
  using E = LN<N>;
  constexpr u32 T = TILE;
  constexpr int RU = ln::has_mul_u<FT> ? SH::RU : -1;
  auto SWZ = [](u32 e) -> u32 { if constexpr (RU >= 0) return e ^ ((e >> 4) & 15u); else return e; };
  extern __shared__ __attribute__((aligned(16))) u32 lds[];
  u32* nqp = lds + (size_t)T * N;
  const u32 k = a.log_n;
  const u32 tiles_per_row = 1u << (k - 10);
  u64 row;
  u32 tile;
  if (FIRST && a.tile_group) {
    const u32 lg = a.tile_group;
    const u32 xcd = blockIdx.x & 7u;
    const u64 qq = blockIdx.x >> 3;
    const u32 sub = (u32)qq & ((1u << lg) - 1);
    const u64 q2 = qq >> lg;
    tile = (((u32)(q2 / a.n_rows) * 8u + xcd) << lg) | sub;
    row = q2 % a.n_rows;
  } else if (tiles_per_row >= 8) {
    const u32 xcd = blockIdx.x & 7u;
    const u64 qq = blockIdx.x >> 3;
    tile = (u32)(qq / a.n_rows) * 8u + xcd;
    row = qq % a.n_rows;
  } else {
    row = blockIdx.x / tiles_per_row;
    tile = blockIdx.x % tiles_per_row;
  }
  const u32 tid = threadIdx.x;
  mem_phase(true);
  const u32 lb = FIRST ? k - S : 0u;
  auto gindex = [&](u32 e) -> u32 {
    if constexpr (FIRST) return ((e >> LBT) << lb) | (tile << LTJ) | (e & ((1u << LBT) - 1));
    else return (tile << S) | e;
  };
  for (u32 i = tid; i < 64 * FT::STRIDE; i += 256) nqp[i] = 0u - a.qp29[i];
  const u32* src = a.src + row * a.src_stride * NL;
  constexpr bool DOUT = N <= 5;
  E xin[4];
#pragma unroll
  for (u32 it = 0; it < 4; it++) {
    const u32 e = tid + 256u * it;
    const u32 g = gindex(e);
    Fe<NL> v;
    if constexpr (FIRST) {
      v = (g < a.n_valid && row * a.src_stride + g < a.n_src_total) ? fe_load<NL>(src + (size_t)g * NL) : fe_zero<NL>();
      if (a.copy_dst != nullptr && g < a.n_valid) fe_store<NL>(a.copy_dst + (row * a.src_stride + g) * NL, v);
    } else {
      v = fe_load<NL>(src + (size_t)g * NL);
    }
    xin[it] = ln::from_packed<FT>(v);
  }
  const u32* cls_pack = pack + (size_t)(FIRST ? tile : 0u) * pi.class_words;
  const bool canon = a.roots29c != nullptr && ((u32)row & a.canon_row_mask) == 0;
  const bool blk0_tile = (FIRST || tile == 0) && a.blk0_gone == 0;
  const bool zero_hi = FIRST && a.n_valid <= (1ull << (k - 1));

  if constexpr (SH::U0 == 1) {
    constexpr u32 half = 1u << (S - 1 + LBT);
    const u32* blk = cls_pack + pi.round_off[0];
#pragma unroll
    for (u32 pp = 0; pp < 2; pp++) {
      const u32 e1 = tid + 256u * pp;
      const E w = pack_get<FT, 2>(blk, SH::period2, canon ? 1u : 0u, e1);
      const E x = xin[pp];
      if (pp == 0) mem_phase(false);
      if (zero_hi) {
        planes_put<FT>(lds, T, SWZ(e1), x);
        planes_put<FT>(lds, T, SWZ(e1 + half), ln::mul<FT>(x, w));
      } else {
        const E y = xin[pp + 2];
        E sum = ln::add(x, y);
        ln::normalize<FT>(sum);
        planes_put<FT>(lds, T, SWZ(e1), sum);
        planes_put<FT>(lds, T, SWZ(e1 + half), ln::mul<FT>(ln::sub(x, y), w));
      }
    }
    mem_phase(true);
    __syncthreads();
  }

  const u32 q = tid;
#pragma unroll
  for (int r = 0; r < SH::NR4; r++) {
    const int u = SH::U0 + 2 * r, hb = S - u - 1;
    const bool last_two = LAST && (r == SH::NR4 - 1);
    const u32 lp = q & ((1u << LBT) - 1), j = q >> LBT;
    const u32 i0 = ((j >> (hb - 1)) << (hb + 1)) | (j & ((1u << (hb - 1)) - 1));
    const u32 e0 = (i0 << LBT) | lp;
    constexpr u32 one = 1u;
    const u32 dq = one << (hb - 1 + LBT);
    const u32 period = one << (hb - 1 + LBT);
    const u32 jl = q & (period - 1);
    const u32* blk = cls_pack + pi.round_off[SH::U0 + r];
    if constexpr (RU >= 0) {
      if (r >= RU && !last_two) {
        const u32 wv = __builtin_amdgcn_readfirstlane(tid >> 6);
        const u32 qu = ((tid & 63u) << 2) | wv;
        const u32 lpu = qu & ((1u << LBT) - 1), ju = qu >> LBT;
        const u32 iu = ((ju >> (hb - 1)) << (hb + 1)) | (ju & ((1u << (hb - 1)) - 1));
        const u32 eu = (iu << LBT) | lpu;
        const u32* wu = cls_pack + pi.u_off + ((r - RU) * 4 + wv) * (3 * U_SLOT<FT>);
        const E x0 = planes_get<FT>(lds, T, SWZ(eu)), x1 = planes_get<FT>(lds, T, SWZ(eu + dq));
        const E x2 = planes_get<FT>(lds, T, SWZ(eu + 2 * dq)), x3 = planes_get<FT>(lds, T, SWZ(eu + 3 * dq));
        mem_phase(false);
        const E b0 = ln::add(x0, x2), b1 = ln::add(x1, x3);
        E c0 = ln::add(b0, b1);
        ln::clamp_apply<FT>(c0, ln::clamp_row<FT>(nqp, ln::clamp_q<FT>(c0.v[N - 1])));
        planes_put<FT>(lds, T, SWZ(eu), c0);
        E d1 = ln::sub(b0, b1);
        ln::normalize<FT>(d1);
        planes_put<FT>(lds, T, SWZ(eu + dq), ln::mul_u<FT>(d1, wu + 2 * U_SLOT<FT>));
        const E b2 = ln::mul_u<FT>(ln::sub(x0, x2), wu);
        const E b3 = ln::mul_u<FT>(ln::sub(x1, x3), wu + U_SLOT<FT>);
        E c2 = ln::add(b2, b3);
        ln::normalize<FT>(c2);
        planes_put<FT>(lds, T, SWZ(eu + 2 * dq), c2);
        planes_put<FT>(lds, T, SWZ(eu + 3 * dq), ln::mul_u<FT>(ln::sub(b2, b3), wu + 2 * U_SLOT<FT>));
        mem_phase(true);
        __syncthreads();
        continue;
      }
    }
    if (u == 0 && zero_hi) {
      const u32 vb = canon ? 3u : 0u;
      const E w0 = pack_get<FT, 6>(blk, period, vb + 0, jl), w2 = pack_get<FT, 6>(blk, period, vb + 2, jl);
      const E w3 = pack_get<FT, 6>(blk, period, vb + 1, jl);
      mem_phase(false);
      if (a.n_valid <= (1ull << (k - 2))) {
        const E x0 = xin[0];
        planes_put<FT>(lds, T, SWZ(e0), x0);
        planes_put<FT>(lds, T, SWZ(e0 + dq), ln::mul<FT>(x0, w2));
        planes_put<FT>(lds, T, SWZ(e0 + 2 * dq), ln::mul<FT>(x0, w0));
        planes_put<FT>(lds, T, SWZ(e0 + 3 * dq), ln::mul<FT>(x0, w3));
      } else {
        const E x0 = xin[0], x1 = xin[1];
        E c0 = ln::add(x0, x1);
        ln::normalize<FT>(c0);
        planes_put<FT>(lds, T, SWZ(e0), c0);
        planes_put<FT>(lds, T, SWZ(e0 + dq), ln::mul<FT>(ln::sub(x0, x1), w2));
        const E t = mul_i<FT>(x1, a);
        planes_put<FT>(lds, T, SWZ(e0 + 2 * dq), ln::mul<FT>(ln::add(x0, t), w0));
        planes_put<FT>(lds, T, SWZ(e0 + 3 * dq), ln::mul<FT>(ln::sub(x0, t), w3));
      }
      mem_phase(true);
      __syncthreads();
      continue;
    }
    const bool from_regs = SH::U0 == 0 && r == 0;
    const E x0 = from_regs ? xin[0] : planes_get<FT>(lds, T, SWZ(e0)), x1 = from_regs ? xin[1] : planes_get<FT>(lds, T, SWZ(e0 + dq));
    const E x2 = from_regs ? xin[2] : planes_get<FT>(lds, T, SWZ(e0 + 2 * dq)), x3 = from_regs ? xin[3] : planes_get<FT>(lds, T, SWZ(e0 + 3 * dq));
    mem_phase(false);
    const E b0 = ln::add(x0, x2), b1 = ln::add(x1, x3);
    E c0 = ln::add(b0, b1);
    if (last_two || from_regs) ln::normalize<FT>(c0);
    else ln::clamp_apply<FT>(c0, ln::clamp_row<FT>(nqp, ln::clamp_q<FT>(c0.v[N - 1])));
    if (!(last_two && DOUT)) planes_put<FT>(lds, T, SWZ(e0), c0);
    if (last_two) {
      E c1 = ln::sub(b0, b1);
      const E b2 = ln::sub(x0, x2);
      const E b3 = mul_i<FT>(ln::sub(x1, x3), a);
      E c2 = ln::add(b2, b3);
      E c3 = ln::sub(b2, b3);
      ln::normalize<FT>(c1); ln::normalize<FT>(c2); ln::normalize<FT>(c3);
      if constexpr (!DOUT) {
        planes_put<FT>(lds, T, SWZ(e0 + dq), c1);
        planes_put<FT>(lds, T, SWZ(e0 + 2 * dq), c2);
        planes_put<FT>(lds, T, SWZ(e0 + 3 * dq), c3);
      } else {
      mem_phase(true);
      u32* dstq = a.dst + row * a.dst_stride * NL + (size_t)((tile << S) | e0) * NL;
      E cc[4] = {c0, c1, c2, c3};
#pragma unroll
      for (int c = 0; c < 4; c++) {
        E x = cc[c];
        ln::clamp_apply<FT>(x, ln::clamp_row<FT>(nqp, ln::clamp_q<FT>(x.v[N - 1])));
        u32 w[NL];
        ln::to_packed<FT>(w, x.v);
        Fe<NL> v;
        if (__any((int)(x.v[N - 1] >= FT::limb(N - 1)))) v = fe_reduce_once<NL>(w, 0u);
        else {
#pragma unroll
          for (int i = 0; i < NL; i++) v.v[i] = w[i];
        }
        if (canon && tile == 0 && e0 + (u32)c < a.mont_prefix) v = fe_canon<NL>(v);
        fe_store<NL>(dstq + (size_t)c * NL, v);
      }
      return;
      }
    } else {
      const bool blk0c = canon && blk0_tile && q < period && (RU < 0 || r < RU);
      if constexpr (RU >= 1) {
        if (r == RU - 1 && blk0c) {
          E kc;
#pragma unroll
          for (int i = 0; i < N; i++) kc.v[i] = i == 0 ? (1u << (N * FT::W - 32 * NL)) : 0u;
          planes_put<FT>(lds, T, SWZ(e0), ln::mul<FT>(c0, kc));
        }
      }
      const u32 vb = blk0c ? 3u : 0u;
      const E w2 = pack_get<FT, 6>(blk, period, vb + 2, jl);
      planes_put<FT>(lds, T, SWZ(e0 + dq), ln::mul<FT>(ln::sub(b0, b1), w2));
      const E t = mul_i<FT>(ln::sub(x1, x3), a);
      const E e2 = ln::sub(x0, x2);
      const E w0 = pack_get<FT, 6>(blk, period, vb + 0, jl), w3 = pack_get<FT, 6>(blk, period, vb + 1, jl);
      planes_put<FT>(lds, T, SWZ(e0 + 2 * dq), ln::mul<FT>(ln::add(e2, t), w0));
      planes_put<FT>(lds, T, SWZ(e0 + 3 * dq), ln::mul<FT>(ln::sub(e2, t), w3));
    }
    mem_phase(true);
    __syncthreads();
  }

  if constexpr (FIRST || N > 5) {
  u32* dst = a.dst + row * a.dst_stride * NL;
#pragma unroll
  for (u32 e = tid; e < T; e += 256) {
    const u32 g = gindex(e);
    E x = planes_get<FT>(lds, T, SWZ(e));
    ln::clamp_apply<FT>(x, ln::clamp_row<FT>(nqp, ln::clamp_q<FT>(x.v[N - 1])));
    u32 w[NL];
    ln::to_packed<FT>(w, x.v);
    Fe<NL> v;
#pragma unroll
    for (int i = 0; i < NL; i++) v.v[i] = w[i];
    if constexpr (LAST) {
      if (__any((int)(x.v[N - 1] >= FT::limb(N - 1)))) v = fe_reduce_once<NL>(w, 0u);
      if (canon && tile == 0 && g < a.mont_prefix) v = fe_canon<NL>(v);
    }
    fe_store<NL>(dst + (size_t)g * NL, v);
  }
  }
}

template <class FT, int S, int LBT>
__global__ void __launch_bounds__(256) ntt_lns_pack_kernel(NttPassArgs a, NttPackInfo pi, u32 n_classes, bool first, u32* pack) {
  using SH = Shape<S, LBT>;
  constexpr u32 n_slots = SH::U0 + SH::NR4;
  constexpr u32 PMAX = 1u << (S - 1 + LBT);
  const u32 k = a.log_n, t0 = a.t0;
  const u32 lb = first ? k - S : 0u;
  const u64 total = (u64)n_classes * n_slots * PMAX;
  for (u64 id = (u64)blockIdx.x * 256 + threadIdx.x; id < total; id += (u64)gridDim.x * 256) {
    const u32 jl = (u32)(id % PMAX), slot = (u32)((id / PMAX) % n_slots), cls = (u32)(id / PMAX / n_slots);
    u32* blk = pack + (size_t)cls * pi.class_words + pi.round_off[slot];
    const u32 lo = first ? (cls << LBT) : 0u;
    if (SH::U0 == 1 && slot == 0) {
      const u32 lp = jl & ((1u << LBT) - 1), i = jl >> LBT;
      const u32 g1 = (i << lb) | lo | lp;
      const u32 gm = (1u << (k - t0 - 1)) - 1;
      pack_put<FT, 2>(blk, SH::period2, 0, jl, tab_entry<FT>(a.roots29, (g1 & gm) << t0));
      pack_put<FT, 2>(blk, SH::period2, 1, jl, tab_entry<FT>(a.roots29c, (g1 & gm) << t0));
      continue;
    }
    const u32 r = slot - SH::U0, u = SH::U0 + 2 * r, hb = S - u - 1, period = 1u << (hb - 1 + LBT);
    const u32 t = t0 + u;
    if (jl >= period || t + 2 == k) continue;
    const u32 gm0 = (1u << (k - t - 1)) - 1;
    const u32 lp = jl & ((1u << LBT) - 1), j = jl >> LBT;
    const u32 i0 = ((j >> (hb - 1)) << (hb + 1)) | (j & ((1u << (hb - 1)) - 1));
    const u32 g0 = (i0 << lb) | lo | lp;
    const u32 ex = (g0 & gm0) << t, half_n = 1u << (k - 1);
    const u32 idx[3] = {ex, 3 * ex, 2 * ex};
    for (u32 v = 0; v < 6; v++) {
      const u32 ix = idx[v % 3];
      LN<FT::N> m = tab_entry<FT>(v < 3 ? a.roots29 : a.roots29c, ix & (half_n - 1));
      if (ix >= half_n) {
        int32_t br = 0;
#pragma unroll
        for (int z = 0; z < FT::N; z++) {
          const int32_t d = (int32_t)FT::limb(z) - (int32_t)m.v[z] - br;
          br = d < 0 ? 1 : 0;
          m.v[z] = z + 1 < FT::N ? (u32)d & ((1u << FT::W) - 1) : (u32)d;
        }
      }
      pack_put<FT, 6>(blk, period, v, jl, m);
    }
  }
}

template <class FT, int S, int LBT>
__global__ void __launch_bounds__(64) ntt_lns_upack_kernel(NttPassArgs a, NttPackInfo pi, u32 n_classes, bool first, u32* pack) {
  using SH = Shape<S, LBT>;
  constexpr int N = FT::N, W = FT::W;
  constexpr u32 M = (1u << W) - 1;
  const u32 k = a.log_n, t0 = a.t0;
  const u32 lb = first ? k - S : 0u;
  const u32 id = blockIdx.x * 64 + threadIdx.x;
  if (id >= n_classes * SH::NRU * 12) return;
  const u32 cls = id / (SH::NRU * 12), ru = (id / 12) % SH::NRU, jl0 = (id % 12) / 3, v = id % 3;
  const u32 r = SH::RU + ru;
  const u32 u = SH::U0 + 2 * r, hb = S - u - 1;
  const u32 t = t0 + u;
  if (t + 2 == k) return;
  const u32 jl = jl0 & (SH::period4(r) - 1);
  const u32 lo = first ? (cls << LBT) : 0u;
  const u32 gm0 = (1u << (k - t - 1)) - 1, gm1 = gm0 >> 1;
  const u32 lp = jl & ((1u << LBT) - 1), j = jl >> LBT;
  const u32 i0 = ((j >> (hb - 1)) << (hb + 1)) | (j & ((1u << (hb - 1)) - 1));
  const u32 g0 = (i0 << lb) | lo | lp;
  const u32 g1 = g0 + (1u << (hb - 1 + lb));
  const u32 idx = v == 0 ? (g0 & gm0) << t : (v == 1 ? (g1 & gm0) << t : (g0 & gm1) << (t + 1));
  const LN<N> w = tab_entry<FT>(a.roots29, idx);
  u32* out = pack + (size_t)cls * pi.class_words + pi.u_off + ((ru * 4 + jl0) * 3 + v) * U_SLOT<FT>;
  for (u32 jj = 0; jj < (u32)N; jj++) {
    LN<N> sh;
#pragma unroll
    for (int z = 0; z < N; z++) sh.v[z] = (u32)z == jj ? 1u : 0u;
    LN<N> x = ln::mul<FT>(sh, w);
    LN<N> tt;
#pragma unroll
    for (int z = 0; z < N; z++) {
      const u32 hz = z + 1 < N ? ((FT::limb(z) >> 1) | ((FT::limb(z + 1) & 1u) << (W - 1))) : (FT::limb(z) >> 1);
      tt.v[z] = x.v[z] + hz;
    }
    ln::normalize<FT>(tt);
    if ((int32_t)tt.v[N - 1] < 0) {
#pragma unroll
      for (int z = 0; z < N; z++) x.v[z] += FT::limb(z);
      ln::normalize<FT>(x);
    }
#pragma unroll
    for (int kk = 0; kk < N; kk++) out[N * kk + jj] = kk + 1 < N ? (x.v[kk] & M) : x.v[kk];
  }
  for (u32 z = N * N; z < U_SLOT<FT>; z++) out[z] = 0;
}

template <class FT, int S, int LBT> NttPackInfo pack_info_t() {
  using SH = Shape<S, LBT>;
  NttPackInfo pi{};
  u32 off = 0, slot = 0;
  if (SH::U0) { pi.round_off[slot++] = off; off += 2 * SH::period2 * FT::N; off = (off + 3) & ~3u; }
  for (int r = 0; r < SH::NR4; r++) { pi.round_off[slot++] = off; off += 6 * SH::period4(r) * FT::N; off = (off + 3) & ~3u; }
  if (ln::has_mul_u<FT> && SH::RU >= 0) { off = (off + U_ALIGN<FT> - 1) & ~(U_ALIGN<FT> - 1); pi.u_off = off; off += SH::NRU * 4 * 3 * U_SLOT<FT>; }
  pi.class_words = off;
  return pi;
}

template <class FT, int S, int LTJ, bool FIRST>
hipError_t launch_t(const NttPassArgs& a, const u32* pack, const NttPackInfo& pi, hipStream_t st) {
  const u64 tiles = ((u64)1 << (a.log_n - 10)) * a.n_rows;
  const size_t lds_bytes = ((size_t)TILE * FT::N + 64 * FT::STRIDE) * 4;
  hipLaunchKernelGGL((ntt_pass_lns_kernel<FT, S, LTJ, FIRST>), dim3((unsigned)tiles), dim3(256), lds_bytes, st, a, pack, pi);
  return hipGetLastError();
}

template <class FT>
__global__ void __launch_bounds__(256) roots_ln_kernel(const u32* roots, u64 n, const u32* rprime, u32* out) {
  const u64 i = (u64)blockIdx.x * 256 + threadIdx.x;
  if (i >= n) return;
  const Fe<FT::NL> c = fe_load<FT::NL>(rprime);
  const Fe<FT::NL> t = fe_mul<FT::NL>(fe_load<FT::NL>(roots + i * FT::NL), c);
  const LN<FT::N> l = ln::from_packed<FT>(t);
#pragma unroll
  for (int k = 0; k < FT::STRIDE; k++) out[i * FT::STRIDE + k] = k < FT::N ? l.v[k] : 0u;
}

#define LNS_FIRST_CASES(X) X(1) X(2) X(3) X(4) X(5) X(6) X(7) X(8) X(9) X(10)

template <class FT> NttPackInfo pack_info_f(uint32_t s, bool first) {
  if (!first) return pack_info_t<FT, 10, 0>();
  switch (s) {
#define X(SV) case SV: return pack_info_t<FT, SV, 10 - SV>();
    LNS_FIRST_CASES(X)
#undef X
  }
  return NttPackInfo{};
}
template <class FT> hipError_t launch_pack_f(const NttPassArgs& a, bool first, const NttPackInfo& pi, uint32_t n_classes, uint32_t* pack, hipStream_t st) {
  const unsigned ugrid = (n_classes * 2 * 12 + 63) / 64;
  if (!first) {
    hipLaunchKernelGGL((ntt_lns_pack_kernel<FT, 10, 0>), dim3(64), dim3(256), 0, st, a, pi, n_classes, false, pack);
    if constexpr (ln::has_mul_u<FT>) hipLaunchKernelGGL((ntt_lns_upack_kernel<FT, 10, 0>), dim3(ugrid), dim3(64), 0, st, a, pi, n_classes, false, pack);
    return hipGetLastError();
  }
  switch (a.s) {
#define X(SV) case SV: hipLaunchKernelGGL((ntt_lns_pack_kernel<FT, SV, 10 - SV>), dim3(2048), dim3(256), 0, st, a, pi, n_classes, true, pack); break;
    LNS_FIRST_CASES(X)
#undef X
    default: return hipErrorInvalidValue;
  }
  if constexpr (ln::has_mul_u<FT>) {
    if (a.s == 8) hipLaunchKernelGGL((ntt_lns_upack_kernel<FT, 8, 2>), dim3(ugrid), dim3(64), 0, st, a, pi, n_classes, true, pack);
    if (a.s == 9) hipLaunchKernelGGL((ntt_lns_upack_kernel<FT, 9, 1>), dim3(ugrid), dim3(64), 0, st, a, pi, n_classes, true, pack);
    if (a.s == 10) hipLaunchKernelGGL((ntt_lns_upack_kernel<FT, 10, 0>), dim3(ugrid), dim3(64), 0, st, a, pi, n_classes, true, pack);
  }
  return hipGetLastError();
}
template <class FT> hipError_t launch_pass_f(const NttPassArgs& a, bool first, const uint32_t* pack, const NttPackInfo& pi, hipStream_t st) {
  if (!first) {
    if (a.s != 10 || a.log_tj != 0 || a.t0 + a.s != a.log_n) return hipErrorInvalidValue;
    return launch_t<FT, 10, 0, false>(a, pack, pi, st);
  }
  if (a.t0 != 0 || a.s + a.log_tj != 10 || (a.s + 10 != a.log_n && a.s + 20 != a.log_n)) return hipErrorInvalidValue;
  switch (a.s) {
#define X(SV) case SV: return launch_t<FT, SV, 10 - SV, true>(a, pack, pi, st);
    LNS_FIRST_CASES(X)
#undef X
  }
  return hipErrorInvalidValue;
}

}

#define LNS_DISPATCH(nl, EXPR)                         \
  switch (nl) {                                        \
    case 2: { using FT = LnField<FT63>; EXPR; }        \
    case 4: { using FT = LnField<FT127>; EXPR; }       \
    case 6: { using FT = LnField<FT191>; EXPR; }       \
    case 8: { using FT = LnField<FT255>; EXPR; }       \
    default: break;                                    \
  }

bool ntt_lns_supported(int nl, uint32_t log_n) { return (nl == 2 || nl == 4 || nl == 6) && log_n >= 11 && log_n <= 20u; }
bool ntt_lns3_supported(int nl, uint32_t log_n) { return (nl == 2 || nl == 4 || nl == 6) && log_n >= 21 && log_n <= 26; }
__global__ void __launch_bounds__(256) lns_subtable_kernel(const u32* tab, u32 shift, u64 n, u32 words, u32* sub) {
  for (u64 id = (u64)blockIdx.x * 256 + threadIdx.x; id < n * words; id += (u64)gridDim.x * 256) {
    const u64 i = id / words, w = id % words;
    sub[i * words + w] = tab[(i << shift) * words + w];
  }
}
hipError_t launch_ntt_lns_subtable(int nl, const uint32_t* tab, uint32_t shift, uint64_t n, uint32_t* sub, hipStream_t st) {
  hipLaunchKernelGGL(lns_subtable_kernel, dim3(2048), dim3(256), 0, st, tab, shift, n, (u32)ntt_lns_stride(nl), sub);
  return hipGetLastError();
}
int ntt_lns_limbs(int nl) { LNS_DISPATCH(nl, return FT::N) return 0; }
int ntt_lns_limb_bits(int nl) { LNS_DISPATCH(nl, return FT::W) return 0; }
int ntt_lns_stride(int nl) { LNS_DISPATCH(nl, return FT::STRIDE) return 0; }

NttPackInfo ntt_lns_pack_info(int nl, uint32_t s, bool first) {
  LNS_DISPATCH(nl, return pack_info_f<FT>(s, first))
  return NttPackInfo{};
}
hipError_t launch_ntt_lns_roots(int nl, const uint32_t* roots, uint64_t n, const uint32_t* rprime, uint32_t* out, hipStream_t st) {
  const dim3 grid((unsigned)((n + 255) / 256));
  LNS_DISPATCH(nl, hipLaunchKernelGGL((roots_ln_kernel<FT>), grid, dim3(256), 0, st, roots, n, rprime, out); return hipGetLastError())
  return hipErrorInvalidValue;
}
hipError_t launch_ntt_lns_pack(int nl, const NttPassArgs& a, bool first, const NttPackInfo& pi, uint32_t n_classes, uint32_t* pack, hipStream_t st) {
  LNS_DISPATCH(nl, return launch_pack_f<FT>(a, first, pi, n_classes, pack, st))
  return hipErrorInvalidValue;
}
hipError_t launch_ntt_pass_lns(int nl, const NttPassArgs& a, bool first, const uint32_t* pack, const NttPackInfo& pi, hipStream_t st) {
  if (a.tile_group && (!first || ((1u << (a.log_n - 10)) >> a.tile_group) < 8)) return hipErrorInvalidValue;
  switch (nl) {
    case 2: return launch_pass_f<LnField<FT63>>(a, first, pack, pi, st);
    case 4: return launch_pass_f<LnField<FT127>>(a, first, pack, pi, st);
    case 6: return launch_pass_f<LnField<FT191>>(a, first, pack, pi, st);
  }
  return hipErrorInvalidValue;
}

}
```

Measured before the change: 7.302 billion.

## Add coset-form two-pass L9S NTT with per-column twiddles moved to last pass

Adds an alternative NTT factorisation for the 255-bit field two-pass path: the first pass uses pure (tile-independent) twiddles shared by all tiles, and the last pass applies coset-dependent twiddles packed per class. It is enabled by default when s0>=6, or forced via LCPC_NTT_FORM. The aim is to shrink the first-pass twiddle pack to a single class and cut twiddle memory traffic, using a new radix-4 last-pass loop and different LDS swizzles. The cost is a larger per-class pack for the last pass and more kernel template instantiations.

New measurement: 7.414 billion, median of 6. 1.02x the previous value.

```diff
diff --git a/lcpc_amd/csrc/ctx.cpp b/lcpc_amd/csrc/ctx.cpp
--- a/lcpc_amd/csrc/ctx.cpp
+++ b/lcpc_amd/csrc/ctx.cpp
@@ -213,15 +213,19 @@
       p.roots29c = sub ? c->d_rootslcs : c->d_rootslc;
       p.mont_prefix = last && c->NL == 2 ? 4u : 0u;
       p.blk0_gone = last && c->NL != 2 && plan[i - 1].a.s >= 8 ? 1u : 0u;
-      p.pack_info = ntt_lns_pack_info(c->NL, p.a.s, p.first);
-      const uint32_t n_classes = p.first ? 1u << (p.a.log_n - 10) : 1u;
+      const bool nf = c->L == 4 && n_pass == 2 && (c->sw_ntt_form == 1 || (c->sw_ntt_form < 0 && s0 >= 6));
+      p.a.form = nf ? 1u : 0u;
+      if (nf && last) p.blk0_gone = 1u;
+      p.pack_info = nf ? ntt_l9s_form_pack_info(p.a.s, p.first) : ntt_lns_pack_info(c->NL, p.a.s, p.first);
+      const uint32_t n_classes = p.first != nf ? 1u << (p.a.log_n - 10) : 1u;
 #ifdef LCPC_TEST_HOOKS
       if (n_pass == 3 && i == 0 && c->sw_test_fail_3pass) return LCPC_ERR_NOMEM;
 #endif
       if ((r = alloc(&p.pack, (size_t)n_classes * p.pack_info.class_words * 4))) return r;
       NttPassArgs pa{};
       pa.roots29 = p.a.roots29; pa.roots29c = p.roots29c; pa.log_n = p.a.log_n; pa.t0 = p.a.t0; pa.s = p.a.s; pa.log_tj = p.a.log_tj;
-      HIPCHK(c, launch_ntt_lns_pack(c->NL, pa, p.first, p.pack_info, n_classes, p.pack, nullptr));
+      if (nf) HIPCHK(c, launch_ntt_l9s_form_pack(pa, p.first, p.pack_info, n_classes, p.pack, nullptr));
+      else HIPCHK(c, launch_ntt_lns_pack(c->NL, pa, p.first, p.pack_info, n_classes, p.pack, nullptr));
     }
     HIPCHK(c, hipDeviceSynchronize());
     return 0;
@@ -570,6 +574,7 @@
   c->f = f; c->L = f->L; c->NL = 2 * f->L;
   if (c->prm.sdig_code == 0) c->prm.sdig_code = 3;
   c->sw_ntt_general = getenv("LCPC_NTT_GENERAL") != nullptr;
+  if (const char* ev = getenv("LCPC_NTT_FORM")) c->sw_ntt_form = !strcmp(ev, "dif") ? 0 : (!strcmp(ev, "coset") ? 1 : -1);
   if (const char* ev = getenv("LCPC_NTT_MID_MAX_MB")) c->sw_ntt_mid_max_mb = (int64_t)strtoull(ev, nullptr, 10);
   if (const char* ev = getenv("LCPC_HOST_STAGE")) c->sw_host_stage = (int32_t)strtol(ev, nullptr, 10);
   c->sw_debug_timing = getenv("LCPC_DEBUG_TIMING") != nullptr;
diff --git a/lcpc_amd/csrc/internal.h b/lcpc_amd/csrc/internal.h
--- a/lcpc_amd/csrc/internal.h
+++ b/lcpc_amd/csrc/internal.h
@@ -216,6 +216,7 @@
 struct lcpc_ctx {
   lcpc_params prm{};
   bool sw_ntt_general = false;
+  int sw_ntt_form = -1;
   int64_t sw_ntt_mid_max_mb = -1;
   bool sw_debug_timing = false;
   bool sw_test_fail_3pass = false;
diff --git a/lcpc_amd/csrc/kernels.h b/lcpc_amd/csrc/kernels.h
--- a/lcpc_amd/csrc/kernels.h
+++ b/lcpc_amd/csrc/kernels.h
@@ -23,6 +23,7 @@
   uint32_t blk0_gone = 0;
   const uint32_t* wq_w = nullptr;
   uint32_t tile_group = 0;
+  uint32_t form = 0;
 };
 hipError_t launch_ntt_pass(int nl, int log_tile, const NttPassArgs& a, hipStream_t st);
 
@@ -34,6 +35,8 @@
 bool ntt_l9s_supported(uint32_t log_n, uint32_t n_passes, int log_tile);
 bool ntt_l9s3_supported(uint32_t log_n);
 hipError_t launch_ntt_pass_l9s(const NttPassArgs& a, bool first, const uint32_t* pack, const NttPackInfo& pi, hipStream_t st);
+NttPackInfo ntt_l9s_form_pack_info(uint32_t s, bool first);
+hipError_t launch_ntt_l9s_form_pack(const NttPassArgs& a, bool first, const NttPackInfo& pi, uint32_t n_classes, uint32_t* pack, hipStream_t st);
 
 bool ntt_lns_supported(int nl, uint32_t log_n);
 bool ntt_lns3_supported(int nl, uint32_t log_n);
diff --git a/lcpc_amd/csrc/ntt_l9s.hip b/lcpc_amd/csrc/ntt_l9s.hip
--- a/lcpc_amd/csrc/ntt_l9s.hip
+++ b/lcpc_amd/csrc/ntt_l9s.hip
@@ -5,7 +5,7 @@
 
 namespace {
 
-template <int S, int LTJ, bool FIRST, bool MID>
+template <int S, int LTJ, bool FIRST, bool MID, bool NF>
 __global__ void __launch_bounds__(256, 4) ntt_pass_l9s_kernel(NttPassArgs a, const u32* __restrict__ pack, NttPackInfo pi) {
   using FT = LnField<FT255>;
   constexpr int NL = 8, LT = S + LTJ, LBT = LTJ;
@@ -13,8 +13,16 @@
   static_assert(LT == 10, "1024-element tiles: one radix-4 quad (two radix-2 pairs) per thread and round");
   static_assert(FIRST || (LTJ == 0 && S % 2 == 0), "the last pass works on contiguous tiles and ends with the trivial stages k-2, k-1");
   using SH = Shape<S, LBT>;
-  constexpr int RU = SH::RU;
-  auto SWZ = [](u32 e) -> u32 { if constexpr (RU >= 0) return e ^ ((e >> 4) & 15u); else return e; };
+  using SP = PureShape<S>;
+  constexpr int RU = NF ? (FIRST ? SP::RU : -1) : SH::RU;
+  constexpr int RC = NF && FIRST ? SP::RC : -1;
+  constexpr bool SWZD = NF ? (LAST || SP::RU >= 0) : RU >= 0;
+  auto SWZ = [](u32 e) -> u32 {
+    if constexpr (NF && LAST) return e ^ (((e >> 4) & 3u) * 5u);
+    else if constexpr (NF && FIRST && SWZD && LBT == 2) return e ^ ((((e >> 4) ^ (e >> 6)) & 3u) << 2);
+    else if constexpr (SWZD) return e ^ ((e >> 4) & 15u);
+    else return e;
+  };
   extern __shared__ __attribute__((aligned(16))) u32 lds[];
   constexpr u32 T = 1u << LT;
   u32* nqp = lds + (size_t)T * 9;
@@ -54,7 +62,7 @@
   if constexpr (LAST && MID) {
     const uint4* t4 = reinterpret_cast<const uint4*>(a.mid + (row << k) * 9 + (size_t)tile * (9 * T));
     uint4* l4 = reinterpret_cast<uint4*>(lds);
-    if constexpr (RU >= 0) {
+    if constexpr (SWZD) {
 #pragma unroll
       for (u32 i = tid; i < 2 * T; i += 256) l4[(i & ~(T - 1)) | SWZ(i & (T - 1))] = t4[i];
 #pragma unroll
@@ -83,8 +91,11 @@
   }
   __builtin_amdgcn_sched_barrier(0);
   }
-  const u32* cls_pack = pack + (size_t)(FIRST ? tile : 0u) * pi.class_words;
+  const u32* cls_pack = pack + (size_t)(FIRST != NF ? tile : 0u) * pi.class_words;
   const bool blk0_tile = (FIRST || tile == 0) && a.blk0_gone == 0;
+  LN<9> k32;
+#pragma unroll
+  for (int i = 0; i < 9; i++) k32.v[i] = i == 0 ? 32u : 0u;
   const bool zero_hi = FIRST && a.n_valid <= (1ull << (k - 1));
   if constexpr (!DIRECT) __syncthreads();
 
@@ -94,17 +105,18 @@
 #pragma unroll
     for (u32 pp = 0; pp < 2; pp++) {
       const u32 e1 = tid + 256u * pp;
-      const LN<9> w = pack_get<FT, 2>(blk, SH::period2, canon ? 1u : 0u, e1);
+      const LN<9> w = NF ? pack_get<FT, 2>(blk, 1u << (S - 1), canon ? 1u : 0u, e1 >> LBT) : pack_get<FT, 2>(blk, SH::period2, canon ? 1u : 0u, e1);
       const LN<9> x = DIRECT ? xin[pp] : planes_get<FT>(lds, T, SWZ(e1));
       if (pp == 0) mem_phase(false);
+      const bool cvs = NF && canon && SH::NR4 <= 1;
       if (zero_hi) {
-        if constexpr (DIRECT) planes_put<FT>(lds, T, SWZ(e1), x);
+        if constexpr (DIRECT) planes_put<FT>(lds, T, SWZ(e1), cvs ? ln::mul<FT>(x, k32) : x);
         planes_put<FT>(lds, T, SWZ(e1 + half), ln::mul<FT>(x, w));
       } else {
         const LN<9> y = DIRECT ? xin[pp + 2] : planes_get<FT>(lds, T, SWZ(e1 + half));
         LN<9> sum = ln::add(x, y);
         ln::normalize<FT>(sum);
-        planes_put<FT>(lds, T, SWZ(e1), sum);
+        planes_put<FT>(lds, T, SWZ(e1), cvs ? ln::mul<FT>(sum, k32) : sum);
         planes_put<FT>(lds, T, SWZ(e1 + half), ln::mul<FT>(ln::sub(x, y), w));
       }
     }
@@ -113,22 +125,112 @@
   }
 
   const u32 q = tid;
+  if constexpr (NF && LAST) {
+#pragma unroll
+    for (int r = 0; r < 5; r++) {
+      const int hb = 9 - 2 * r;
+      const u32 D = 1u << (hb - 1);
+      const u32 m = q >> (hb - 1);
+      const u32 e0 = (m << (hb + 1)) | (q & (D - 1));
+      const bool from_regs = DIRECT && r == 0;
+      LN<9> x0 = from_regs ? xin[0] : planes_get<FT>(lds, T, SWZ(e0));
+      const LN<9> x1 = from_regs ? xin[1] : planes_get<FT>(lds, T, SWZ(e0 + D));
+      const LN<9> x2 = from_regs ? xin[2] : planes_get<FT>(lds, T, SWZ(e0 + 2 * D)), x3 = from_regs ? xin[3] : planes_get<FT>(lds, T, SWZ(e0 + 3 * D));
+      LN<9> p1, p2, p3;
+      if (r < 2) {
+        const u32 sb = r == 0 ? 0u : (u32)__builtin_amdgcn_readfirstlane(tid >> 6);
+        const u32* wu = cls_pack + pi.u_off + ((u32)r * 4 + sb) * (3 * U_SLOT<FT>);
+        mem_phase(false);
+        if (!from_regs) ln::clamp_apply<FT>(x0, ln::clamp_row<FT>(nqp, ln::clamp_q<FT>(x0.v[8])));
+        p2 = ln::mul_u<FT>(x2, wu + U_SLOT<FT>);
+        p1 = ln::mul_u<FT>(x1, wu);
+        p3 = ln::mul_u<FT>(x3, wu + 2 * U_SLOT<FT>);
+      } else {
+        const u32* blk = cls_pack + pi.round_off[r];
+        const LN<9> w1 = pack_get<FT, 3>(blk, coset_sets(r), 0, m), w2 = pack_get<FT, 3>(blk, coset_sets(r), 1, m);
+        const LN<9> w3 = pack_get<FT, 3>(blk, coset_sets(r), 2, m);
+        mem_phase(false);
+        ln::clamp_apply<FT>(x0, ln::clamp_row<FT>(nqp, ln::clamp_q<FT>(x0.v[8])));
+        p2 = ln::mul<FT>(x2, w2);
+        p1 = ln::mul<FT>(x1, w1);
+        p3 = ln::mul<FT>(x3, w3);
+      }
+      const LN<9> s02 = ln::add(x0, p2), d02 = ln::sub(x0, p2), s13 = ln::add(p1, p3);
+      LN<9> y0 = ln::add(s02, s13), y1 = ln::sub(s02, s13);
+      ln::normalize<FT>(y0);
+      const LN<9> t = ln::mul_u<FT>(ln::sub(p1, p3), a.wq_w);
+      LN<9> y2 = ln::add(d02, t), y3 = ln::sub(d02, t);
+      if (r == 0 || r == 4) { ln::normalize<FT>(y1); ln::normalize<FT>(y2); ln::normalize<FT>(y3); }
+      mem_phase(true);
+      if (r < 4) {
+        planes_put<FT>(lds, T, SWZ(e0), y0);
+        planes_put<FT>(lds, T, SWZ(e0 + D), y1);
+        planes_put<FT>(lds, T, SWZ(e0 + 2 * D), y2);
+        planes_put<FT>(lds, T, SWZ(e0 + 3 * D), y3);
+        __syncthreads();
+      } else {
+        u32* dstq = a.dst + row * a.dst_stride * NL + (size_t)((tile << S) | e0) * NL;
+        LN<9> cc[4] = {y0, y1, y2, y3};
+#pragma unroll
+        for (int c = 0; c < 4; c++) {
+          LN<9> x = cc[c];
+          ln::clamp_apply<FT>(x, ln::clamp_row<FT>(nqp, ln::clamp_q<FT>(x.v[8])));
+          u32 w[8];
+          ln::to_packed<FT>(w, x.v);
+          Fe<NL> v;
+#pragma unroll
+          for (int i = 0; i < 8; i++) v.v[i] = w[i];
+          if (__any((int)(x.v[8] >= FT::limb(8)))) v = fe_reduce_once<8>(w);
+          fe_store<NL>(dstq + (size_t)c * NL, v);
+        }
+      }
+    }
+    return;
+  }
 #pragma unroll
   for (int r = 0; r < SH::NR4; r++) {
     const int u = SH::U0 + 2 * r, hb = S - u - 1;
     const bool last_two = LAST && (r == SH::NR4 - 1);
+    const bool triv = NF && FIRST && (r == SH::NR4 - 1);
     const u32 lp = q & ((1u << LBT) - 1), j = q >> LBT;
     const u32 i0 = ((j >> (hb - 1)) << (hb + 1)) | (j & ((1u << (hb - 1)) - 1));
     const u32 e0 = (i0 << LBT) | lp;
     constexpr u32 one = 1u;
     const u32 dq = one << (hb - 1 + LBT);
-    const u32 period = one << (hb - 1 + LBT);
-    const u32 jl = q & (period - 1);
+    const u32 period = NF ? one << (hb - 1) : one << (hb - 1 + LBT);
+    const u32 jl = NF ? j & (period - 1) : q & (period - 1);
     const u32* blk = cls_pack + pi.round_off[SH::U0 + r];
+    if (triv) {
+      const bool fr = DIRECT && SH::U0 == 0 && r == 0;
+      const LN<9> x0 = fr ? xin[0] : planes_get<FT>(lds, T, SWZ(e0)), x1 = fr ? xin[1] : planes_get<FT>(lds, T, SWZ(e0 + dq));
+      const LN<9> x2 = fr ? xin[2] : planes_get<FT>(lds, T, SWZ(e0 + 2 * dq)), x3 = fr ? xin[3] : planes_get<FT>(lds, T, SWZ(e0 + 3 * dq));
+      mem_phase(false);
+      const LN<9> b0 = ln::add(x0, x2), b1 = ln::add(x1, x3);
+      LN<9> c0 = ln::add(b0, b1), c1 = ln::sub(b0, b1);
+      const LN<9> b2 = ln::sub(x0, x2);
+      const LN<9> t = ln::mul_u<FT>(ln::sub(x1, x3), a.wq_w);
+      LN<9> c2 = ln::add(b2, t), c3 = ln::sub(b2, t);
+      ln::normalize<FT>(c1); ln::normalize<FT>(c2); ln::normalize<FT>(c3);
+      if (RC < 0 && SH::U0 == 0 && canon) {
+        ln::normalize<FT>(c0);
+        c0 = ln::mul<FT>(c0, k32); c1 = ln::mul<FT>(c1, k32); c2 = ln::mul<FT>(c2, k32); c3 = ln::mul<FT>(c3, k32);
+      } else if (fr) {
+        ln::normalize<FT>(c0);
+      } else {
+        ln::clamp_apply<FT>(c0, ln::clamp_row<FT>(nqp, ln::clamp_q<FT>(c0.v[8])));
+      }
+      planes_put<FT>(lds, T, SWZ(e0), c0);
+      planes_put<FT>(lds, T, SWZ(e0 + dq), c1);
+      planes_put<FT>(lds, T, SWZ(e0 + 2 * dq), c2);
+      planes_put<FT>(lds, T, SWZ(e0 + 3 * dq), c3);
+      mem_phase(true);
+      __syncthreads();
+      continue;
+    }
     if constexpr (RU >= 0) {
       if (r >= RU && !last_two) {
         const u32 wv = __builtin_amdgcn_readfirstlane(tid >> 6);
-        const u32 qu = ((tid & 63u) << 2) | wv;
+        const u32 qu = NF ? (((((tid & 63u) >> LBT) << 2) | wv) << LBT) | (tid & ((1u << LBT) - 1)) : ((tid & 63u) << 2) | wv;
         const u32 lpu = qu & ((1u << LBT) - 1), ju = qu >> LBT;
         const u32 iu = ((ju >> (hb - 1)) << (hb + 1)) | (ju & ((1u << (hb - 1)) - 1));
         const u32 eu = (iu << LBT) | lpu;
@@ -146,7 +248,8 @@
         const LN<9> b2 = ln::mul_u<FT>(ln::sub(x0, x2), wu);
         const LN<9> b3 = ln::mul_u<FT>(ln::sub(x1, x3), wu + U_SLOT<FT>);
         LN<9> c2 = ln::add(b2, b3);
-        ln::normalize<FT>(c2);
+        if constexpr (NF) ln::clamp_apply<FT>(c2, ln::clamp_row<FT>(nqp, ln::clamp_q<FT>(c2.v[8])));
+        else ln::normalize<FT>(c2);
         planes_put<FT>(lds, T, SWZ(eu + 2 * dq), c2);
         planes_put<FT>(lds, T, SWZ(eu + 3 * dq), ln::mul_u<FT>(ln::sub(b2, b3), wu + 2 * U_SLOT<FT>));
         mem_phase(true);
@@ -158,9 +261,10 @@
       const u32 vb = canon ? 3u : 0u;
       const LN<9> w0 = pack_get<FT, 6>(blk, period, vb + 0, jl), w3 = pack_get<FT, 6>(blk, period, vb + 1, jl), w2 = pack_get<FT, 6>(blk, period, vb + 2, jl);
       mem_phase(false);
+      const bool cv0 = NF && canon && r == RC;
       if (a.n_valid <= (1ull << (k - 2))) {
         const LN<9> x0 = DIRECT ? xin[0] : planes_get<FT>(lds, T, SWZ(e0));
-        if constexpr (DIRECT) planes_put<FT>(lds, T, SWZ(e0), x0);
+        if constexpr (DIRECT) planes_put<FT>(lds, T, SWZ(e0), cv0 ? ln::mul<FT>(x0, k32) : x0);
         planes_put<FT>(lds, T, SWZ(e0 + dq), ln::mul<FT>(x0, w2));
         planes_put<FT>(lds, T, SWZ(e0 + 2 * dq), ln::mul<FT>(x0, w0));
         planes_put<FT>(lds, T, SWZ(e0 + 3 * dq), ln::mul<FT>(x0, w3));
@@ -168,7 +272,7 @@
         const LN<9> x0 = DIRECT ? xin[0] : planes_get<FT>(lds, T, SWZ(e0)), x1 = DIRECT ? xin[1] : planes_get<FT>(lds, T, SWZ(e0 + dq));
         LN<9> c0 = ln::add(x0, x1);
         ln::normalize<FT>(c0);
-        planes_put<FT>(lds, T, SWZ(e0), c0);
+        planes_put<FT>(lds, T, SWZ(e0), cv0 ? ln::mul<FT>(c0, k32) : c0);
         planes_put<FT>(lds, T, SWZ(e0 + dq), ln::mul<FT>(ln::sub(x0, x1), w2));
         const LN<9> t = ln::mul_u<FT>(x1, a.wq_w);
         planes_put<FT>(lds, T, SWZ(e0 + 2 * dq), ln::mul<FT>(ln::add(x0, t), w0));
@@ -212,12 +316,9 @@
       if (from_regs) ln::normalize<FT>(c0);
       else ln::clamp_apply<FT>(c0, ln::clamp_row<FT>(nqp, ln::clamp_q<FT>(c0.v[8])));
       planes_put<FT>(lds, T, SWZ(e0), c0);
-      const bool blk0c = canon && blk0_tile && q < period && (RU < 0 || r < RU);
-      if constexpr (RU >= 1) {
-        if (r == RU - 1 && blk0c) {
-          LN<9> k32;
-#pragma unroll
-          for (int i = 0; i < 9; i++) k32.v[i] = i == 0 ? 32u : 0u;
+      const bool blk0c = NF ? canon && q < dq : canon && blk0_tile && q < period && (RU < 0 || r < RU);
+      if constexpr (NF ? RC >= 0 : RU >= 1) {
+        if (r == (NF ? RC : RU - 1) && blk0c) {
           planes_put<FT>(lds, T, SWZ(e0), ln::mul<FT>(c0, k32));
         }
       }
@@ -265,20 +366,21 @@
   }
 }
 
-template <int S, int LTJ, bool FIRST, bool MID>
+template <int S, int LTJ, bool FIRST, bool MID, bool NF>
 hipError_t launch_tm(const NttPassArgs& a, const u32* pack, const NttPackInfo& pi, hipStream_t st) {
   constexpr int LT = S + LTJ;
   const u64 tiles = ((u64)1 << (a.log_n - LT)) * a.n_rows;
   const size_t lds_bytes = (((size_t)1 << LT) * 9 + 64 * LnField<FT255>::STRIDE) * 4;
-  hipError_t e = hipFuncSetAttribute(reinterpret_cast<const void*>(&ntt_pass_l9s_kernel<S, LTJ, FIRST, MID>),
+  hipError_t e = hipFuncSetAttribute(reinterpret_cast<const void*>(&ntt_pass_l9s_kernel<S, LTJ, FIRST, MID, NF>),
                                      hipFuncAttributeMaxDynamicSharedMemorySize, (int)lds_bytes);
   if (e != hipSuccess) return e;
-  hipLaunchKernelGGL((ntt_pass_l9s_kernel<S, LTJ, FIRST, MID>), dim3((unsigned)tiles), dim3(256), lds_bytes, st, a, pack, pi);
+  hipLaunchKernelGGL((ntt_pass_l9s_kernel<S, LTJ, FIRST, MID, NF>), dim3((unsigned)tiles), dim3(256), lds_bytes, st, a, pack, pi);
   return hipGetLastError();
 }
 template <int S, int LTJ, bool FIRST>
 hipError_t launch_t(const NttPassArgs& a, const u32* pack, const NttPackInfo& pi, hipStream_t st) {
-  return a.mid ? launch_tm<S, LTJ, FIRST, true>(a, pack, pi, st) : launch_tm<S, LTJ, FIRST, false>(a, pack, pi, st);
+  if (a.form) return a.mid ? launch_tm<S, LTJ, FIRST, true, true>(a, pack, pi, st) : launch_tm<S, LTJ, FIRST, false, true>(a, pack, pi, st);
+  return a.mid ? launch_tm<S, LTJ, FIRST, true, false>(a, pack, pi, st) : launch_tm<S, LTJ, FIRST, false, false>(a, pack, pi, st);
 }
 
 }
@@ -296,6 +398,7 @@
     return launch_t<10, 0, false>(a, pack, pi, st);
   }
   if (a.t0 != 0 || a.s + a.log_tj != 10 || (a.s + 10 != a.log_n && a.s + 20 != a.log_n)) return hipErrorInvalidValue;
+  if (a.form && a.s + 10 != a.log_n) return hipErrorInvalidValue;
   if (a.tile_group && ((1u << (a.log_n - 10)) >> a.tile_group) < 8) return hipErrorInvalidValue;
   switch (a.s) {
 #define X(SV) case SV: return launch_t<SV, 10 - SV, true>(a, pack, pi, st);
diff --git a/lcpc_amd/csrc/ntt_ln_dev.h b/lcpc_amd/csrc/ntt_ln_dev.h
--- a/lcpc_amd/csrc/ntt_ln_dev.h
+++ b/lcpc_amd/csrc/ntt_ln_dev.h
@@ -11,6 +11,15 @@
   static constexpr int RU = NR4 >= 4 ? 3 : -1;
   static constexpr int NRU = RU < 0 ? 0 : NR4 - RU;
 };
+template <int S> struct PureShape {
+  static constexpr int U0 = S & 1;
+  static constexpr int NR4 = S / 2;
+  static constexpr u32 sets(int r) { return 1u << (S - U0 - 2 * r - 2); }
+  static constexpr int RU = NR4 >= 3 ? NR4 - 2 : -1;
+  static constexpr int RC = NR4 >= 3 ? NR4 - 3 : (NR4 == 2 ? 0 : -1);
+};
+constexpr u32 coset_sets(int r) { return 1u << (2 * r); }
+
 template <class FT> constexpr u32 U_SLOT = (FT::N * FT::N + 31) & ~31u;
 template <class FT> constexpr u32 U_ALIGN = FT::N == 9 ? 4u : 16u;
 
diff --git a/lcpc_amd/csrc/ntt_lns.hip b/lcpc_amd/csrc/ntt_lns.hip
--- a/lcpc_amd/csrc/ntt_lns.hip
+++ b/lcpc_amd/csrc/ntt_lns.hip
@@ -251,6 +251,19 @@
   }
 }
 
+template <class FT> LCPC_DEV LN<FT::N> tab_entry_neg(const u32* tab, u32 ix, u32 half_n) {
+  LN<FT::N> m = tab_entry<FT>(tab, ix & (half_n - 1));
+  if (ix >= half_n) {
+    int32_t br = 0;
+#pragma unroll
+    for (int z = 0; z < FT::N; z++) {
+      const int32_t d = (int32_t)FT::limb(z) - (int32_t)m.v[z] - br;
+      br = d < 0 ? 1 : 0;
+      m.v[z] = z + 1 < FT::N ? (u32)d & ((1u << FT::W) - 1) : (u32)d;
+    }
+  }
+  return m;
+}
 template <class FT, int S, int LBT>
 __global__ void __launch_bounds__(256) ntt_lns_pack_kernel(NttPassArgs a, NttPackInfo pi, u32 n_classes, bool first, u32* pack) {
   using SH = Shape<S, LBT>;
@@ -280,28 +293,38 @@
     const u32 g0 = (i0 << lb) | lo | lp;
     const u32 ex = (g0 & gm0) << t, half_n = 1u << (k - 1);
     const u32 idx[3] = {ex, 3 * ex, 2 * ex};
-    for (u32 v = 0; v < 6; v++) {
-      const u32 ix = idx[v % 3];
-      LN<FT::N> m = tab_entry<FT>(v < 3 ? a.roots29 : a.roots29c, ix & (half_n - 1));
-      if (ix >= half_n) {
-        int32_t br = 0;
-#pragma unroll
-        for (int z = 0; z < FT::N; z++) {
-          const int32_t d = (int32_t)FT::limb(z) - (int32_t)m.v[z] - br;
-          br = d < 0 ? 1 : 0;
-          m.v[z] = z + 1 < FT::N ? (u32)d & ((1u << FT::W) - 1) : (u32)d;
-        }
-      }
-      pack_put<FT, 6>(blk, period, v, jl, m);
-    }
-  }
-}
-
+    for (u32 v = 0; v < 6; v++) pack_put<FT, 6>(blk, period, v, jl, tab_entry_neg<FT>(v < 3 ? a.roots29 : a.roots29c, idx[v % 3], half_n));
+  }
+}
+
+template <class FT> LCPC_DEV void upack_write(const LN<FT::N>& w, u32* out) {
+  constexpr int N = FT::N, W = FT::W;
+  constexpr u32 M = (1u << W) - 1;
+  for (u32 jj = 0; jj < (u32)N; jj++) {
+    LN<N> sh;
+#pragma unroll
+    for (int z = 0; z < N; z++) sh.v[z] = (u32)z == jj ? 1u : 0u;
+    LN<N> x = ln::mul<FT>(sh, w);
+    LN<N> tt;
+#pragma unroll
+    for (int z = 0; z < N; z++) {
+      const u32 hz = z + 1 < N ? ((FT::limb(z) >> 1) | ((FT::limb(z + 1) & 1u) << (W - 1))) : (FT::limb(z) >> 1);
+      tt.v[z] = x.v[z] + hz;
+    }
+    ln::normalize<FT>(tt);
+    if ((int32_t)tt.v[N - 1] < 0) {
+#pragma unroll
+      for (int z = 0; z < N; z++) x.v[z] += FT::limb(z);
+      ln::normalize<FT>(x);
+    }
+#pragma unroll
+    for (int kk = 0; kk < N; kk++) out[N * kk + jj] = kk + 1 < N ? (x.v[kk] & M) : x.v[kk];
+  }
+  for (u32 z = N * N; z < U_SLOT<FT>; z++) out[z] = 0;
+}
 template <class FT, int S, int LBT>
 __global__ void __launch_bounds__(64) ntt_lns_upack_kernel(NttPassArgs a, NttPackInfo pi, u32 n_classes, bool first, u32* pack) {
   using SH = Shape<S, LBT>;
-  constexpr int N = FT::N, W = FT::W;
-  constexpr u32 M = (1u << W) - 1;
   const u32 k = a.log_n, t0 = a.t0;
   const u32 lb = first ? k - S : 0u;
   const u32 id = blockIdx.x * 64 + threadIdx.x;
@@ -319,29 +342,46 @@
   const u32 g0 = (i0 << lb) | lo | lp;
   const u32 g1 = g0 + (1u << (hb - 1 + lb));
   const u32 idx = v == 0 ? (g0 & gm0) << t : (v == 1 ? (g1 & gm0) << t : (g0 & gm1) << (t + 1));
-  const LN<N> w = tab_entry<FT>(a.roots29, idx);
-  u32* out = pack + (size_t)cls * pi.class_words + pi.u_off + ((ru * 4 + jl0) * 3 + v) * U_SLOT<FT>;
-  for (u32 jj = 0; jj < (u32)N; jj++) {
-    LN<N> sh;
-#pragma unroll
-    for (int z = 0; z < N; z++) sh.v[z] = (u32)z == jj ? 1u : 0u;
-    LN<N> x = ln::mul<FT>(sh, w);
-    LN<N> tt;
-#pragma unroll
-    for (int z = 0; z < N; z++) {
-      const u32 hz = z + 1 < N ? ((FT::limb(z) >> 1) | ((FT::limb(z + 1) & 1u) << (W - 1))) : (FT::limb(z) >> 1);
-      tt.v[z] = x.v[z] + hz;
-    }
-    ln::normalize<FT>(tt);
-    if ((int32_t)tt.v[N - 1] < 0) {
-#pragma unroll
-      for (int z = 0; z < N; z++) x.v[z] += FT::limb(z);
-      ln::normalize<FT>(x);
-    }
-#pragma unroll
-    for (int kk = 0; kk < N; kk++) out[N * kk + jj] = kk + 1 < N ? (x.v[kk] & M) : x.v[kk];
-  }
-  for (u32 z = N * N; z < U_SLOT<FT>; z++) out[z] = 0;
+  const LN<FT::N> w = tab_entry<FT>(a.roots29, idx);
+  upack_write<FT>(w, pack + (size_t)cls * pi.class_words + pi.u_off + ((ru * 4 + jl0) * 3 + v) * U_SLOT<FT>);
+}
+
+using F255 = LnField<FT255>;
+__global__ void __launch_bounds__(64) l9s_pure_upack_kernel(NttPassArgs a, NttPackInfo pi, u32 u, u32* pack) {
+  const u32 id = threadIdx.x;
+  if (id >= 12) return;
+  const u32 jl0 = id / 3, v = id % 3;
+  const u32 k = a.log_n, lb = k - a.s, hb = a.s - u - 1;
+  const u32 gm0 = (1u << (k - u - 1)) - 1, gm1 = gm0 >> 1;
+  const u32 g0 = jl0 << lb, g1 = g0 + (1u << (hb - 1 + lb));
+  const u32 idx = v == 0 ? (g0 & gm0) << u : (v == 1 ? (g1 & gm0) << u : (g0 & gm1) << (u + 1));
+  upack_write<F255>(tab_entry<F255>(a.roots29, idx), pack + pi.u_off + (jl0 * 3 + v) * U_SLOT<F255>);
+}
+LCPC_DEV u32 coset_exp(u32 k, u32 cls, u32 r, u32 m) {
+  const u32 S = k - 10;
+  const u32 k1 = __brev(cls) >> (32 - S);
+  const u32 rm = r ? __brev(m) >> (32 - 2 * r) : 0u;
+  return (k1 + (rm << S)) << (8 - 2 * r);
+}
+__global__ void __launch_bounds__(256) l9s_coset_pack_kernel(NttPassArgs a, NttPackInfo pi, u32 n_classes, u32* pack) {
+  const u32 k = a.log_n, half_n = 1u << (k - 1);
+  const u64 total = (u64)n_classes * 336;
+  for (u64 id = (u64)blockIdx.x * 256 + threadIdx.x; id < total; id += (u64)gridDim.x * 256) {
+    const u32 cls = (u32)(id / 336), x = (u32)(id % 336);
+    const u32 r = x < 16 ? 2u : (x < 80 ? 3u : 4u), m = x < 16 ? x : (x < 80 ? x - 16 : x - 80);
+    const u32 E = coset_exp(k, cls, r, m);
+    u32* blk = pack + (size_t)cls * pi.class_words + pi.round_off[r];
+    for (u32 v = 0; v < 3; v++) pack_put<F255, 3>(blk, coset_sets(r), v, m, tab_entry_neg<F255>(a.roots29, (v + 1) * E, half_n));
+  }
+}
+__global__ void __launch_bounds__(64) l9s_coset_upack_kernel(NttPassArgs a, NttPackInfo pi, u32 n_classes, u32* pack) {
+  const u32 k = a.log_n, half_n = 1u << (k - 1);
+  const u32 id = blockIdx.x * 64 + threadIdx.x;
+  if (id >= n_classes * 15) return;
+  const u32 cls = id / 15, x = id % 15;
+  const u32 r = x < 3 ? 0u : 1u, m = x < 3 ? 0u : (x - 3) / 3, v = x % 3;
+  const u32 E = coset_exp(k, cls, r, m);
+  upack_write<F255>(tab_entry_neg<F255>(a.roots29, (v + 1) * E, half_n), pack + (size_t)cls * pi.class_words + pi.u_off + ((r * 4 + m) * 3 + v) * U_SLOT<F255>);
 }
 
 template <class FT, int S, int LBT> NttPackInfo pack_info_t() {
@@ -376,6 +416,24 @@
 
 #define LNS_FIRST_CASES(X) X(1) X(2) X(3) X(4) X(5) X(6) X(7) X(8) X(9) X(10)
 
+NttPackInfo form_pack_info(uint32_t s, bool first) {
+  NttPackInfo pi{};
+  u32 off = 0;
+  if (first) {
+    const u32 u0 = s & 1, nr4 = s / 2;
+    u32 slot = 0;
+    if (u0) { pi.round_off[slot++] = off; off += 2 * (1u << (s - 1)) * 9; off = (off + 3) & ~3u; }
+    for (u32 r = 0; r < nr4; r++) { pi.round_off[slot++] = off; off += 6 * (1u << (s - u0 - 2 * r - 2)) * 9; off = (off + 3) & ~3u; }
+    if (nr4 >= 3) { pi.u_off = off; off += 4 * 3 * U_SLOT<F255>; }
+  } else {
+    for (u32 r = 2; r < 5; r++) { pi.round_off[r] = off; off += 3 * coset_sets(r) * 9; }
+    pi.u_off = off;
+    off += 2 * 4 * 3 * U_SLOT<F255>;
+  }
+  pi.class_words = off;
+  return pi;
+}
+
 template <class FT> NttPackInfo pack_info_f(uint32_t s, bool first) {
   if (!first) return pack_info_t<FT, 10, 0>();
   switch (s) {
@@ -430,6 +488,24 @@
     default: break;                                    \
   }
 
+NttPackInfo ntt_l9s_form_pack_info(uint32_t s, bool first) { return form_pack_info(s, first); }
+hipError_t launch_ntt_l9s_form_pack(const NttPassArgs& a, bool first, const NttPackInfo& pi, uint32_t n_classes, uint32_t* pack, hipStream_t st) {
+  if (a.log_n < 11 || a.log_n > 20 || a.s != (first ? a.log_n - 10 : 10u)) return hipErrorInvalidValue;
+  if (!first) {
+    hipLaunchKernelGGL(l9s_coset_pack_kernel, dim3(n_classes >= 1024 ? 1344u : (n_classes * 336 + 255) / 256), dim3(256), 0, st, a, pi, n_classes, pack);
+    hipLaunchKernelGGL(l9s_coset_upack_kernel, dim3((n_classes * 15 + 63) / 64), dim3(64), 0, st, a, pi, n_classes, pack);
+    return hipGetLastError();
+  }
+  if (n_classes != 1) return hipErrorInvalidValue;
+  switch (a.s) {
+#define X(SV) case SV: hipLaunchKernelGGL((ntt_lns_pack_kernel<F255, SV, 0>), dim3(4), dim3(256), 0, st, a, pi, 1u, true, pack); break;
+    LNS_FIRST_CASES(X)
+#undef X
+  }
+  const u32 u0 = a.s & 1, nr4 = a.s / 2;
+  if (nr4 >= 3) hipLaunchKernelGGL(l9s_pure_upack_kernel, dim3(1), dim3(64), 0, st, a, pi, u0 + 2 * (nr4 - 2), pack);
+  return hipGetLastError();
+}
 bool ntt_lns_supported(int nl, uint32_t log_n) { return (nl == 2 || nl == 4 || nl == 6) && log_n >= 11 && log_n <= 20u; }
 bool ntt_lns3_supported(int nl, uint32_t log_n) { return (nl == 2 || nl == 4 || nl == 6) && log_n >= 21 && log_n <= 26; }
 __global__ void __launch_bounds__(256) lns_subtable_kernel(const u32* tab, u32 shift, u64 n, u32 words, u32* sub) {
```
